# AO33/HiC_Genome_Assembler

Hardware: AMD Instinct MI355X
Metric: Part1+Part2 wall-clock (s) and bins/s on N x N contact map (higher is better)
Workload: dtype f64

## Files before the change

hic_genome_assembler_amd/csrc/api.hip:

```cpp
#include <hip/hip_runtime.h>

#include <algorithm>
#include <cmath>
#include <cstdarg>
#include <climits>
#include <cstdio>
#include <cstdlib>
#include <cstring>
#include <numeric>
#include <string>
#include <type_traits>
#include <unordered_map>
#include <functional>
#include <chrono>
#include <vector>

#include "../../include/hicmi.h"
#include "hicmi_internal.h"
#include "devbuf.h"
#include "hyper.h"

using namespace hicmi;

static thread_local std::string g_err;

static int fail(int code, const char* fmt, ...)
{
    char buf[512];
    va_list ap;
    va_start(ap, fmt);
    vsnprintf(buf, sizeof(buf), fmt, ap);
    va_end(ap);
    g_err = buf;
    return code;
}

namespace hicmi { int set_error(int code, const char* msg) { return fail(code, "%s", msg); } }

#define HIPCHK(expr)                                                                              \
    do {                                                                                          \
        hipError_t _e = (expr);                                                                   \
        if (_e != hipSuccess) return fail(HICMI_EHIP, "%s: %s", #expr, hipGetErrorString(_e));     \
    } while (0)

enum Family { F_ROW_SUMS, F_BUILD_W, F_NNCHAIN, F_SORT, F_RANK_INVERT, F_CUT_COUNT, F_HYPER_FLAGS, F_P2_SELECT,
              F_P2_TOTAL, F_P2_SCORE, F_P2_EXACT, F_P2_INSERT, F_P2_WINDOW_G, F_P2_WINDOW_DELTA, F_PLOT, F_PRESORT, F_RANK_RELABEL,
              F_RANK_TIED, F_P2_WINDOW_FLOPS, F_COUNT };
static const char* kFamilyNames[F_COUNT] = {"row_sums", "build_w", "nnchain", "sort_rows", "rank_invert",
                                            "cut_count", "hyper_flags", "p2_select", "p2_total", "p2_score",
                                            "p2_score_exact", "p2_score_insert", "p2_window_G", "p2_window_delta", "plot",
                                            "presort_rows", "rank_relabel", "rank_rows_tied",
                                            "p2_window_G_flops"};

constexpr int kBaseSlabs = 256;

struct TimedRegion { int fam; hipEvent_t a, b; };

template <typename H, hipError_t (*Destroy)(H)>
struct Handle {
    H h = nullptr;
    Handle() = default;
    Handle(const Handle&) = delete;
    ~Handle() { if (h) (void)Destroy(h); }
    operator H() const { return h; }
};
using StreamHandle = Handle<hipStream_t, hipStreamDestroy>;
using EventHandle = Handle<hipEvent_t, hipEventDestroy>;
struct TimingEvents {
    std::vector<TimedRegion> regions;
    std::vector<hipEvent_t> pool;
    TimingEvents() = default;
    TimingEvents(const TimingEvents&) = delete;
    ~TimingEvents()
    {
        for (auto& r : regions) { (void)hipEventDestroy(r.a); (void)hipEventDestroy(r.b); }
        for (auto e : pool) (void)hipEventDestroy(e);
    }
};

struct hicmi_ctx {
    int device = 0;
    StreamHandle stream;
    StreamHandle stream2; EventHandle ev_fork, ev_join;
    TimingEvents tev;
    int probed_xcc = 0;
    int64_t n = 0, ldc = 0;
    double* dC = nullptr;
    bool own_c = false;
    DevBuf<double> c_own;
    DevBuf<double> d_np, d_seq;
    bool have_sums = false;
    int64_t shard_first = 0, shard_stride = 1;
    DevBuf<double> dW, dW2; int64_t ldw = 0; int64_t w_rows = 0;
    DevBuf<unsigned char> d_size;
    DevBuf<int> d_chain, d_status;
    DevBuf<double> d_zraw;
    std::vector<double> zraw;
    DevBuf<int32_t> d_order;
    DevBuf<uint16_t> dR, dRank; int64_t ldr = 0; int64_t r_rows = 0;
    DevBuf<unsigned char> d_sort_scratch;
    bool have_rank = false;
    DevBuf<uint16_t> dRankS;
    DevBuf<int32_t> d_ident;
    DevBuf<unsigned char> d_ties;
    DevBuf<uint16_t> d_tie_bits; int64_t ld_bits = 0;
    DevBuf<int32_t> d_row_list;
    int64_t scan_first_batch = 0, scan_last_improved = 0;
    int64_t presort_tied_rows = 0;
    int presort_used = 0;
    int64_t presort_n = 0;
    bool presort_dealt = false;
    DevBuf<int32_t> d_x; DevBuf<uint8_t> d_sig;
    DevBuf<unsigned char> d_scan_multi;
    int64_t cached_start = -1;
    DevBuf<double> d_tmp;
    DevBuf<double> dM2; int64_t n2 = 0, ld2 = 0;
    DevBuf<int32_t> d_sel;
    DevBuf<double> d_H;
    DevBuf<int32_t> d_perms;
    DevBuf<double> d_scores;
    DevBuf<double> d_partial;
    DevBuf<double> d_T;
    DevBuf<int32_t> d_scaf_start, d_scaf_len; int64_t n_scaf = 0;
    std::vector<int32_t> h_scaf_start, h_scaf_len;
    DevBuf<int32_t> d_arr_packed;
    std::vector<int32_t> h_arr_packed;
    std::vector<int32_t> h_arr_id, h_arr_pos; std::vector<uint8_t> h_arr_rev;
    DevBuf<int32_t> d_pos2sel; int64_t n_arr = 0;
    DevBuf<int8_t> d_orders; DevBuf<uint8_t> d_orients;
    int tab_k = 0; int64_t n_orders = 0, n_orients = 0;
    std::vector<int8_t> h_orders; std::vector<uint8_t> h_orients;
    std::vector<int32_t> h_pos2sel;
    uint64_t arr_version = 0;
    uint64_t cur_lit_version = ~0ull; double cur_lit_total = 0.0, cur_lit_value = 0.0;
    double cache_total = 0.0; bool cache_valid = false;
    std::unordered_map<std::string, double> exact_cache;
    DevBuf<double> d_G;
    DevBuf<double> d_delta;
    DevBuf<WindowBatchEntry> d_wb;
    int near_min_k = 7;
    DevBuf<unsigned char> d_wnear;
    DevBuf<int32_t> d_arr_packed2;
    DevBuf<int32_t> d_pos2sel2;
    DevBuf<double> d_ins_T;
    DevBuf<double> d_ins_partial;
    DevBuf<unsigned char> d_ins_blob;
    DevBuf<InsStep> d_ins_steps;
    DevBuf<SupRec> d_sup_recs;
    DevBuf<BrkRec> d_brk_recs;
    DevBuf<InvRec> d_inv_recs;
    DevBuf<int32_t> d_gs_lists;
    DevBuf<double> d_gs_sums;
    DevBuf<unsigned char> d_jn_lists;
    DevBuf<double> d_jn_sums;
    DevBuf<double> d_ice;
    DevBuf<uint8_t> d_ice_mask;
    struct HmmSlot { DevBuf<double> d_x; int64_t T = 0, ld = 0, D = 0; };
    HmmSlot hslot[HICMI_HMM_MAX_SLOTS]; int hcur = 0;
    double* d_hx = nullptr; int64_t hmm_T = 0, hmm_ld = 0, hmm_D = 0;
    DevBuf<unsigned char> d_hmulti;
    DevBuf<int32_t> d_horder;
    DevBuf<double> d_hwork;
    DevBuf<int32_t> d_hlab;
    DevBuf<uint8_t> d_hbt;
    DevBuf<double> d_hpart;
    DevBuf<double> d_hsmall;
    DevBuf<double> d_hhist;
    DevBuf<int> d_hst;
    DevBuf<double> d_lvA; int64_t lv_m = 0;
    DevBuf<double> d_lvvec;
    DevBuf<int32_t> d_lvrows;
    DevBuf<unsigned char> d_lvwork;
    DevBuf<double> map_cells; int64_t map_m = 0, map_res = 0, map_pairs = 0;
    DevBuf<int32_t> d_map_first;
    std::vector<int32_t> map_first; std::vector<int64_t> map_size;
    DevBuf<unsigned char> d_map_chunk;
    DevBuf<unsigned char> d_map_lift; LiftTables map_lift; std::vector<int32_t> map_lift_seq;
    DevBuf<unsigned char> d_stat_lift;
    DevBuf<unsigned long long> d_stat_out;
    DevBuf<unsigned long long> span_marks;
    DevBuf<unsigned char> d_span_lift; LiftTables span_lift; SpanGrid span_grid;
    DevBuf<int64_t> d_span_first;
    std::vector<int64_t> span_size, span_seq_first;
    int64_t span_pairs = 0;
    DevBuf<unsigned long long> ends_table; int64_t ends_cells = 0;
    DevBuf<unsigned char> d_ends_lift; LiftTables ends_lift; EndsGrid ends_grid;
    DevBuf<int32_t> d_ends_rank;
    std::vector<int64_t> ends_size;
    DevBuf<unsigned long long> anchor_table; int64_t anchor_cells = 0;
    DevBuf<unsigned char> d_anchor_lift; LiftTables anchor_lift; AnchorGrid anchor_grid;
    DevBuf<int64_t> d_anchor_first;
    DevBuf<int32_t> d_anchor_target;
    std::vector<int64_t> anchor_size;
    DevBuf<int32_t> d_pairs_scaf_a, d_pairs_scaf_b;
    DevBuf<int64_t> d_pairs_pos_a, d_pairs_pos_b;
    DevBuf<unsigned long long> d_pairs_intra;
    DevBuf<long long> d_pairs_work;
    PinBuf<unsigned long long> pin_pairs_len;
    int64_t pairs_len = 0;
    std::vector<int64_t> pairs_size;
    DevBuf<int32_t> d_plot_order;
    DevBuf<unsigned char> d_plot_work;
    DevBuf<double> d_plot_img;
    PinBuf<char> pin_up; size_t pin_up_off = 0;
    PinBuf<char> pin_down;

    int timing = 0;
    double ms[F_COUNT] = {0}; int64_t launches[F_COUNT] = {0}; double bytes[F_COUNT] = {0};
    double nn_scans = 0, nn_scan_cols = 0, nn_cache_hits = 0, nn_merges = 0; int64_t nn_retries = 0;
};

namespace {
hipError_t sync_stream(hicmi_ctx* c);

struct Timed {
    hicmi_ctx* c; int fam; hipEvent_t a = nullptr, b = nullptr; hipStream_t st;
    Timed(hicmi_ctx* ctx, int f, double algo_bytes, hipStream_t on_stream = nullptr) : c(ctx), fam(f), st(on_stream ? on_stream : ctx->stream)
    {
        c->launches[f]++; c->bytes[f] += algo_bytes;
        if (!on()) return;
        a = grab(); b = grab();
        hipEventRecord(a, st);
    }
    bool on() const { return c->timing == 1 || (c->timing == 2 && (fam <= F_RANK_INVERT || fam >= F_PRESORT)); }
    ~Timed()
    {
        if (!on()) return;
        hipEventRecord(b, st);
        c->tev.regions.push_back({fam, a, b});
    }
    hipEvent_t grab()
    {
        if (!c->tev.pool.empty()) { hipEvent_t e = c->tev.pool.back(); c->tev.pool.pop_back(); return e; }
        hipEvent_t e; hipEventCreate(&e); return e;
    }
};

int resolve_timing(hicmi_ctx* c)
{
    if (c->tev.regions.empty()) return HICMI_OK;
    HIPCHK(sync_stream(c));
    if (c->stream2) HIPCHK(hipStreamSynchronize(c->stream2));
    int dropped = 0, dropped_fam = 0;
    hipError_t dropped_err = hipSuccess;
    for (auto& r : c->tev.regions) {
        float ms = 0.f;
        const hipError_t e = hipEventElapsedTime(&ms, r.a, r.b);
        if (e == hipSuccess) c->ms[r.fam] += ms;
        else if (dropped++ == 0) { dropped_fam = r.fam; dropped_err = e; }
        c->tev.pool.push_back(r.a); c->tev.pool.push_back(r.b);
    }
    c->tev.regions.clear();
    if (dropped)
        return fail(HICMI_EHIP, "hipEventElapsedTime failed for %d timed region(s), the first of family %s: %s", dropped,
                    kFamilyNames[dropped_fam], hipGetErrorString(dropped_err));
    return HICMI_OK;
}


hipError_t sync_stream(hicmi_ctx* c)
{
    hipError_t e = hipStreamSynchronize(c->stream);
    c->pin_up_off = 0;
    return e;
}

int upload(hicmi_ctx* c, void* dst, const void* src, size_t bytes)
{
    if (bytes == 0) return HICMI_OK;
    const size_t need = (bytes + 63) & ~(size_t)63;
    if (c->pin_up_off + need > (size_t)c->pin_up.capacity()) {
        HIPCHK(sync_stream(c));
        if (need > (size_t)c->pin_up.capacity()) HIPCHK(c->pin_up.reserve((int64_t)std::max<size_t>(need * 2, (size_t)1 << 20)));
    }
    char* slot = c->pin_up + c->pin_up_off;
    memcpy(slot, src, bytes);
    c->pin_up_off += need;
    HIPCHK(hipMemcpyAsync(dst, slot, bytes, hipMemcpyHostToDevice, c->stream));
    return HICMI_OK;
}

int ensure_pin_down(hicmi_ctx* c, size_t bytes)
{
    if (bytes > (size_t)c->pin_down.capacity()) HIPCHK(c->pin_down.reserve((int64_t)std::max<size_t>(bytes * 2, (size_t)1 << 20)));
    return HICMI_OK;
}

int download(hicmi_ctx* c, void* dst, const void* src, size_t bytes)
{
    if (bytes == 0) { HIPCHK(sync_stream(c)); return HICMI_OK; }
    int rc_pin = ensure_pin_down(c, bytes);
    if (rc_pin) return rc_pin;
    HIPCHK(hipMemcpyAsync(c->pin_down, src, bytes, hipMemcpyDeviceToHost, c->stream));
    HIPCHK(sync_stream(c));
    memcpy(dst, c->pin_down, bytes);
    return HICMI_OK;
}

int no_memory(size_t bytes, hipError_t e)
{
    return fail(HICMI_ENOMEM, "hipMalloc" "(%lld bytes): %s", (long long)bytes, hipGetErrorString(e));
}

template <typename T>
int ensure(DevBuf<T>& buf, int64_t need)
{
    const hipError_t e = buf.reserve(need);
    return e == hipSuccess ? HICMI_OK : no_memory(DevBuf<T>::bytes_for(need), e);
}

template <typename... Args>
int ensure_all(Args&&... args)
{
    size_t failed_bytes = 0;
    const hipError_t e = reserve_all(&failed_bytes, args...);
    return e == hipSuccess ? HICMI_OK : no_memory(failed_bytes, e);
}

int check_candidate_bins(int64_t n_bins)
{
    if (n_bins * (int64_t)sizeof(int32_t) > 160 * 1024) return fail(HICMI_EUNSUPPORTED, "candidate longer than 40960 bins");
    return HICMI_OK;
}

void drop_matrix_state(hicmi_ctx* c)
{
    c->c_own.reset();
    c->dC = nullptr; c->own_c = false; c->n = 0; c->ldc = 0;
    c->d_np.reset(); c->d_seq.reset(); c->have_sums = false;
    c->have_rank = false; c->cached_start = -1; c->n2 = 0;
    if (c->presort_n && c->stream2) (void)hipStreamSynchronize(c->stream2);
    c->presort_n = 0;
}

int alloc_sums(hicmi_ctx* c)
{
    return ensure_all(c->d_np, c->n, c->d_seq, c->n);
}

int compute_sums(hicmi_ctx* c)
{
    if (c->have_sums) return HICMI_OK;
    if (!c->dC) return fail(HICMI_EINVAL, "no contact matrix set");
    {
        Timed t(c, F_ROW_SUMS, 2.0 * 8.0 * (double)c->n * (double)c->n);
        launch_row_sums(c->dC, c->ldc, (int)c->n, c->d_np, c->d_seq, 0, 1, c->stream);
    }
    HIPCHK(hipGetLastError());
    c->have_sums = true;
    return HICMI_OK;
}

int own_matrix(hicmi_ctx* c, DevBuf<double>&& made, int64_t n)
{
    drop_matrix_state(c);
    c->c_own = std::move(made);
    c->dC = c->c_own; c->own_c = true; c->n = n; c->ldc = n;
    int rc = alloc_sums(c);
    return rc ? rc : compute_sums(c);
}

int check_job_context(hicmi_ctx* const* ctxs, int64_t j)
{
    if (!ctxs[j] || !ctxs[0] || ctxs[j]->device != ctxs[0]->device) return fail(HICMI_EINVAL, "contexts must share one device");
    for (int64_t q = 0; q < j; q++) if (ctxs[q] == ctxs[j]) return fail(HICMI_EINVAL, "one context per chromosome");
    return HICMI_OK;
}
}

extern "C" {

int hicmi_abi_version(void) { return HICMI_ABI_VERSION; }
const char* hicmi_last_error(void) { return g_err.c_str(); }

int hicmi_device_count(int* count)
{
    if (!count) return fail(HICMI_EINVAL, "count is NULL");
    int n = 0;
    hipError_t e = hipGetDeviceCount(&n);
    if (e != hipSuccess) { *count = 0; return fail(HICMI_EHIP, "hipGetDeviceCount: %s", hipGetErrorString(e)); }
    *count = n;
    return HICMI_OK;
}

int hicmi_create(int device, hicmi_ctx** out)
{
    if (!out) return fail(HICMI_EINVAL, "out is NULL");
    *out = nullptr;
    int n = 0;
    hipError_t e = hipGetDeviceCount(&n);
    if (e != hipSuccess || n <= 0)
        return fail(HICMI_EHIP, "no HIP device available (%s): libhicmi has no CPU fallback",
                    e != hipSuccess ? hipGetErrorString(e) : "device count 0");
    if (device < 0 || device >= n) return fail(HICMI_EINVAL, "device %d out of range (0..%d)", device, n - 1);
    HIPCHK(hipSetDevice(device));
    hicmi_ctx* c = new hicmi_ctx();
    c->device = device;
    hipError_t se = hipStreamCreateWithFlags(&c->stream.h, hipStreamNonBlocking);
    if (se != hipSuccess) { delete c; return fail(HICMI_EHIP, "hipStreamCreate: %s", hipGetErrorString(se)); }
    c->probed_xcc = nnchain_probe_xcc(c->stream);
    if (const char* dd = getenv("HICMI_P2_DEVICE_DECIDE")) {
        if (!strcmp(dd, "off")) c->near_min_k = INT_MAX;
        else if (atoi(dd) >= 1) c->near_min_k = atoi(dd);
    }
    *out = c;
    return HICMI_OK;
}

int hicmi_destroy(hicmi_ctx* c)
{
    if (!c) return HICMI_OK;
    (void)hipSetDevice(c->device);
    (void)hipStreamSynchronize(c->stream);
    if (c->stream2) (void)hipStreamSynchronize(c->stream2);
    delete c;
    return HICMI_OK;
}

int hicmi_stream(hicmi_ctx* c, void** stream_out)
{
    if (!c || !stream_out) return fail(HICMI_EINVAL, "NULL argument");
    *stream_out = (void*)c->stream;
    return HICMI_OK;
}

int hicmi_synchronize(hicmi_ctx* c)
{
    if (!c) return fail(HICMI_EINVAL, "NULL context");
    HIPCHK(sync_stream(c));
    return HICMI_OK;
}

int hicmi_set_contacts_host(hicmi_ctx* c, const double* contacts, int64_t n)
{
    if (!c || !contacts || n < 1) return fail(HICMI_EINVAL, "bad arguments");
    if (n > 65536) return fail(HICMI_EUNSUPPORTED, "n = %lld > 65536 bins: rank matrix is uint16 in this version", (long long)n);
    HIPCHK(hipSetDevice(c->device));
    drop_matrix_state(c);
    int rc = ensure(c->c_own, n * n);
    if (rc) return rc;
    c->n = n; c->ldc = n; c->dC = c->c_own; c->own_c = true;
    HIPCHK(hipMemcpyAsync(c->dC, contacts, sizeof(double) * (size_t)n * (size_t)n, hipMemcpyHostToDevice, c->stream));
    HIPCHK(sync_stream(c));
    return alloc_sums(c);
}

int hicmi_set_contacts_host_f32(hicmi_ctx* c, const float* contacts, int64_t n)
{
    if (!c || !contacts || n < 1) return fail(HICMI_EINVAL, "bad arguments");
    if (n > 65536) return fail(HICMI_EUNSUPPORTED, "n = %lld > 65536 bins: rank matrix is uint16 in this version", (long long)n);
// ... 2652 lines not shown

void pick_first_strict_max(const std::vector<int64_t>& near, const std::vector<double>& near_fast, const std::vector<double>& lit,
                           double floor, int64_t* pick_out, double* best_out, double* pick_fast_out)
{
    double best = floor; int64_t pick = -1; size_t pick_q = 0;
    for (size_t q = 0; q < near.size(); q++) if (lit[q] > best) { best = lit[q]; pick = near[q]; pick_q = q; }
    *pick_out = pick; *best_out = best;
    if (pick >= 0) *pick_fast_out = near_fast[pick_q];
}

int decide_from_near(hicmi_ctx* c, int64_t first, int64_t k, double total, double floor, double cur_fast, int64_t c0,
                     const std::vector<int64_t>& near, const std::vector<double>& near_fast, int64_t* pick_out,
                     double* best_out, double* pick_fast_out)
{
    const int64_t S = (int64_t)c->h_arr_id.size();
    *pick_out = -1; *best_out = floor; *pick_fast_out = cur_fast;
    if (near.empty()) return HICMI_OK;
    int rc;
    double lit_c0 = 0.0; bool have_c0 = false;
    if (k != S) {
        for (int64_t cand : near) if (cand == c0) have_c0 = true;
        if (have_c0) {
            if (c->cur_lit_version != c->arr_version || c->cur_lit_total != total) {
                std::vector<std::vector<int32_t>> one(1, c->h_pos2sel);
                std::vector<double> v;
                rc = literal_scores(c, one, total, v);
                if (rc) return rc;
                c->cur_lit_version = c->arr_version; c->cur_lit_total = total; c->cur_lit_value = v[0];
            }
            lit_c0 = c->cur_lit_value;
            if (near.size() == 1) {
                if (lit_c0 > floor) { *pick_out = c0; *best_out = lit_c0; *pick_fast_out = near_fast[0]; }
                return HICMI_OK;
            }
        }
    }
    std::vector<int64_t> others;
    for (int64_t cand : near) if (!(have_c0 && cand == c0)) others.push_back(cand);
    std::vector<std::vector<int32_t>> rows;
    near_rows(c, first, k, others, rows);
    std::vector<double> lit_others;
    rc = literal_scores(c, rows, total, lit_others);
    if (rc) return rc;
    std::vector<double> lit(near.size());
    for (size_t q = 0, o = 0; q < near.size(); q++) lit[q] = (have_c0 && near[q] == c0) ? lit_c0 : lit_others[o++];
    pick_first_strict_max(near, near_fast, lit, floor, pick_out, best_out, pick_fast_out);
    return HICMI_OK;
}

int decide_from_delta(hicmi_ctx* c, int64_t first, int64_t k, double total, double floor, double& cur_fast,
                      const double* delta, int64_t* pick_out, double* best_out, double* pick_fast_out)
{
    const int64_t S = (int64_t)c->h_arr_id.size();
    const int64_t n_ord = c->n_orders, n_ori = c->n_orients, n_cand = n_ord * n_ori;
    *pick_out = -1; *best_out = floor; *pick_fast_out = cur_fast;
    const int64_t c0 = window_c0(c, first, k);
    if (c0 < 0) return fail(HICMI_EINVAL, "current orientation not in the orientation table");
    std::vector<double> fast((size_t)n_cand);
    int rc;
    if (k == S) for (int64_t i = 0; i < n_cand; i++) fast[(size_t)i] = delta[(size_t)i] / total;
    else {
        if (std::isnan(cur_fast)) { rc = hicmi_p2_arrangement_score(c, total, &cur_fast); if (rc) return rc; }
        for (int64_t i = 0; i < n_cand; i++) fast[(size_t)i] = cur_fast + (delta[(size_t)i] - delta[(size_t)c0]) / total;
    }
    std::vector<int64_t> near;
    short_list(fast, floor, near);
    std::vector<double> near_fast(near.size());
    for (size_t q = 0; q < near.size(); q++) near_fast[q] = fast[(size_t)near[q]];
    return decide_from_near(c, first, k, total, floor, cur_fast, c0, near, near_fast, pick_out, best_out, pick_fast_out);
}

const int64_t kNearHead = 16;

struct NearPending { int64_t count = 0, cap = 0, head = 0; size_t off_cnt = 0, off_list = 0, host_list = 0; };

int window_near_enqueue(hicmi_ctx* c, int64_t first0, int64_t count, int64_t k, double total, double floor, double& cur_fast,
                        int64_t cap, NearPending& p)
{
    std::vector<WindowBatchEntry> wb;
    BatchCost bc;
    int rc = fill_batch(c, first0, count, k, wb, bc);
    if (rc) return rc;
    if (k > 8 || cap < 1 || cap > (1 << 24)) return fail(HICMI_EINVAL, "short lists take k <= 8 and 1 <= cap <= 2^24");
    const int64_t S = (int64_t)c->h_arr_id.size();
    for (int64_t wdx = 0; wdx < count; wdx++) {
        const int64_t c0 = window_c0(c, first0 + wdx, k);
        if (c0 < 0) return fail(HICMI_EINVAL, "current orientation not in the orientation table");
        wb[(size_t)wdx].c0 = (int32_t)c0;
    }
    if (k != S && std::isnan(cur_fast)) { rc = hicmi_p2_arrangement_score(c, total, &cur_fast); if (rc) return rc; }
    HIPCHK(hipSetDevice(c->device));
    const int n_blocks = window_near_blocks((int)c->n_orders);
    const size_t off_cnt = (size_t)count * (size_t)n_blocks * sizeof(double);
    const size_t off_list = off_cnt + (((size_t)count * sizeof(int32_t) + 15) & ~(size_t)15);
    const size_t bytes = off_list + (size_t)count * (size_t)cap * sizeof(NearEntry);
    rc = ensure(c->d_G, count * window_table_doubles((int)k));
    if (!rc) rc = ensure(c->d_wnear, (int64_t)bytes);
    if (!rc) rc = ensure(c->d_wb, count);
    if (rc) return rc;
    rc = upload(c, c->d_wb, wb.data(), sizeof(WindowBatchEntry) * (size_t)count);
    if (rc) return rc;
    int32_t* d_count = reinterpret_cast<int32_t*>(c->d_wnear + off_cnt);
    NearEntry* d_list = reinterpret_cast<NearEntry*>(c->d_wnear + off_list);
    {
        c->launches[F_P2_WINDOW_FLOPS]++; c->bytes[F_P2_WINDOW_FLOPS] += bc.g_flops;
        Timed t(c, F_P2_WINDOW_G, bc.g_bytes);
        launch_p2_window_near(c->dM2, c->ld2, c->d_pos2sel, (int)c->n_arr, (int)k, c->d_wb, wb.data(), (int)count, bc.max_m,
                              c->d_orders, c->d_orients, (int)c->n_orders, (int)c->n_orients, c->d_H, c->d_G, k == S ? 1 : 0,
                              total, cur_fast, floor, kNearTop, reinterpret_cast<double*>(c->d_wnear.get()), d_count,
                              d_list, (int)cap, c->stream);
    }
    HIPCHK(hipGetLastError());
    p.count = count; p.cap = cap; p.head = std::min<int64_t>(kNearHead, cap); p.off_cnt = off_cnt; p.off_list = off_list;
    p.host_list = off_list - off_cnt;
    const size_t row = (size_t)p.head * sizeof(NearEntry);
    rc = ensure_pin_down(c, p.host_list + row * (size_t)count);
    if (rc) return rc;
    if (count == 1)
        HIPCHK(hipMemcpyAsync(c->pin_down, d_count, p.host_list + row, hipMemcpyDeviceToHost, c->stream));
    else {
        HIPCHK(hipMemcpyAsync(c->pin_down, d_count, sizeof(int32_t) * (size_t)count, hipMemcpyDeviceToHost, c->stream));
        HIPCHK(hipMemcpy2DAsync(c->pin_down + p.host_list, row, d_list, (size_t)cap * sizeof(NearEntry), row, (size_t)count,
                                hipMemcpyDeviceToHost, c->stream));
    }
    return HICMI_OK;
}

int window_near_collect(hicmi_ctx* c, const NearPending& p, std::vector<int64_t>& n_near,
                        std::vector<std::vector<int64_t>>& near, std::vector<std::vector<double>>& near_fast)
{
    const int64_t count = p.count, cap = p.cap;
    HIPCHK(sync_stream(c));
    std::vector<int32_t> cnt((size_t)count);
    memcpy(cnt.data(), c->pin_down, sizeof(int32_t) * (size_t)count);
    n_near.assign((size_t)count, 0); near.assign((size_t)count, {}); near_fast.assign((size_t)count, {});
    int64_t widest = 0;
    for (int64_t w = 0; w < count; w++) {
        n_near[(size_t)w] = cnt[(size_t)w];
        if (cnt[(size_t)w] <= cap) widest = std::max<int64_t>(widest, cnt[(size_t)w]);
    }
    if (widest == 0) return HICMI_OK;
    size_t row = (size_t)p.head * sizeof(NearEntry);
    const char* lists = c->pin_down + p.host_list;
    if (widest > p.head) {
        row = (size_t)widest * sizeof(NearEntry);
        int rc = ensure_pin_down(c, row * (size_t)count);
        if (rc) return rc;
        HIPCHK(hipMemcpy2DAsync(c->pin_down, row, c->d_wnear + p.off_list, (size_t)cap * sizeof(NearEntry), row, (size_t)count,
                                hipMemcpyDeviceToHost, c->stream));
        HIPCHK(sync_stream(c));
        lists = c->pin_down;
    }
    std::vector<NearEntry> ent;
    for (int64_t w = 0; w < count; w++) {
        const int64_t m = cnt[(size_t)w];
        if (m < 1 || m > cap) continue;
        const NearEntry* src = reinterpret_cast<const NearEntry*>(lists + row * (size_t)w);
        ent.assign(src, src + m);
        std::sort(ent.begin(), ent.end(), [](const NearEntry& a, const NearEntry& b) { return a.cand < b.cand; });
        near[(size_t)w].resize((size_t)m); near_fast[(size_t)w].resize((size_t)m);
        for (int64_t q = 0; q < m; q++) { near[(size_t)w][(size_t)q] = ent[(size_t)q].cand; near_fast[(size_t)w][(size_t)q] = ent[(size_t)q].fast; }
    }
    return HICMI_OK;
}

int window_near_batch(hicmi_ctx* c, int64_t first0, int64_t count, int64_t k, double total, double floor, double& cur_fast,
                      int64_t cap, std::vector<int64_t>& n_near, std::vector<std::vector<int64_t>>& near,
                      std::vector<std::vector<double>>& near_fast)
{
    NearPending p;
    int rc = window_near_enqueue(c, first0, count, k, total, floor, cur_fast, cap, p);
    if (rc) return rc;
    return window_near_collect(c, p, n_near, near, near_fast);
}

const int64_t kNearCap = 4096;

int check_window_call(hicmi_ctx* c, int64_t first, int64_t k)
{
    const int64_t S = (int64_t)c->h_arr_id.size();
    if (c->n_arr < 1 || S < 1) return fail(HICMI_EINVAL, "hicmi_p2_set_arrangement has not run");
    if (k != c->tab_k || c->h_orders.empty()) return fail(HICMI_EINVAL, "hicmi_p2_window_tables has not been called for k = %lld", (long long)k);
    if (first < 0 || first + k > S) return fail(HICMI_EINVAL, "window out of range");
    for (int64_t j = 0; j < k; j++) if (c->h_orders[(size_t)j] != j) return fail(HICMI_EINVAL, "orders[0] must be the identity");
    return HICMI_OK;
}
}

int hicmi_p2_decide_window(hicmi_ctx* c, int64_t first, int64_t k, double total, double floor, double cur_fast,
                           int64_t* pick_out, double* best_out, double* pick_fast_out)
{
    if (!c || !pick_out || !best_out || !pick_fast_out) return fail(HICMI_EINVAL, "NULL argument");
    int rc = check_window_call(c, first, k);
    if (rc) return rc;
    use_total(c, total);
    if (k >= c->near_min_k) {
        std::vector<int64_t> n_near; std::vector<std::vector<int64_t>> near; std::vector<std::vector<double>> near_fast;
        rc = window_near_batch(c, first, 1, k, total, floor, cur_fast, kNearCap, n_near, near, near_fast);
        if (rc) return rc;
        if (n_near[0] <= kNearCap)
            return decide_from_near(c, first, k, total, floor, cur_fast, window_c0(c, first, k), near[0], near_fast[0],
                                    pick_out, best_out, pick_fast_out);
    }
    std::vector<double> delta((size_t)(c->n_orders * c->n_orients));
    rc = window_batch(c, first, 1, k, delta.data());
    if (rc) return rc;
    return decide_from_delta(c, first, k, total, floor, cur_fast, delta.data(), pick_out, best_out, pick_fast_out);
}

int hicmi_p2_window_shortlist(hicmi_ctx* c, int64_t first, int64_t count, int64_t k, double total, double floor,
                              double cur_fast, int64_t cap, int64_t* n_near_out, int64_t* idx_out, double* fast_out)
{
    if (!c || !n_near_out || !idx_out || !fast_out || count < 1) return fail(HICMI_EINVAL, "bad arguments");
    int rc = check_window_call(c, first, k);
    if (rc) return rc;
    std::vector<int64_t> n_near; std::vector<std::vector<int64_t>> near; std::vector<std::vector<double>> near_fast;
    rc = window_near_batch(c, first, count, k, total, floor, cur_fast, cap, n_near, near, near_fast);
    if (rc) return rc;
    for (int64_t w = 0; w < count; w++) {
        n_near_out[w] = n_near[(size_t)w];
        for (size_t q = 0; q < near[(size_t)w].size(); q++) {
            idx_out[w * cap + (int64_t)q] = near[(size_t)w][q];
            fast_out[w * cap + (int64_t)q] = near_fast[(size_t)w][q];
        }
    }
    return HICMI_OK;
}

int hicmi_p2_decide_insertion(hicmi_ctx* c, const int32_t* ids, const uint8_t* rev, int64_t S, int32_t new_id,
                              int32_t new_rev_now, int64_t* gap_out, int32_t* rev_out, double* best_out)
{
    if (!c || !ids || !rev || !gap_out || !rev_out || !best_out || S < 1) return fail(HICMI_EINVAL, "bad arguments");
    if (c->n_scaf < 1) return fail(HICMI_EINVAL, "hicmi_p2_layout has not run");
    if (new_id < 0 || new_id >= c->n_scaf) return fail(HICMI_EINVAL, "new scaffold out of range");
    *gap_out = -1; *rev_out = 0; *best_out = 0.0;
    std::vector<int32_t> ids2(ids, ids + S); ids2.push_back(new_id);
    std::vector<uint8_t> rev2(rev, rev + S); rev2.push_back(new_rev_now ? 1 : 0);
    int rc = hicmi_p2_set_arrangement(c, ids2.data(), rev2.data(), S + 1);
    if (rc) return rc;
    double total = 0.0;
    rc = hicmi_p2_arrangement_total(c, &total);
    if (rc) return rc;
    use_total(c, total);
    rc = hicmi_p2_set_arrangement(c, ids, rev, S);
    if (rc) return rc;
    const int64_t gaps = S + 1;
    std::vector<double> by_gap_rev((size_t)(2 * gaps));
    rc = hicmi_p2_score_insertions(c, new_id, total, by_gap_rev.data());
    if (rc) return rc;
    std::vector<double> fast((size_t)(2 * gaps));
    std::vector<int32_t> tag_rev((size_t)(2 * gaps));
    int32_t o = new_rev_now ? 1 : 0;
    for (int64_t i = 0; i < gaps; i++) {
        tag_rev[(size_t)(2 * i)] = o; tag_rev[(size_t)(2 * i + 1)] = o ^ 1;
        fast[(size_t)(2 * i)] = by_gap_rev[(size_t)(2 * i + o)];
        fast[(size_t)(2 * i + 1)] = by_gap_rev[(size_t)(2 * i + (o ^ 1))];
        o ^= 1;
    }
    std::vector<int64_t> near;
    short_list(fast, 0.0, near);
    if (near.empty()) return HICMI_OK;
    const int32_t st = c->h_scaf_start[(size_t)new_id], ln = c->h_scaf_len[(size_t)new_id];
    std::vector<std::vector<int32_t>> rows(near.size());
    for (size_t q = 0; q < near.size(); q++) {
        const int64_t g = near[q] / 2;
        const int32_t r = tag_rev[(size_t)near[q]];
        const int P = c->h_arr_pos[(size_t)g];
        std::vector<int32_t>& row = rows[q];
        row.reserve((size_t)(c->n_arr + ln));
        row.insert(row.end(), c->h_pos2sel.begin(), c->h_pos2sel.begin() + P);
        if (r) for (int32_t e = 0; e < ln; e++) row.push_back(st + ln - 1 - e);
        else   for (int32_t e = 0; e < ln; e++) row.push_back(st + e);
        row.insert(row.end(), c->h_pos2sel.begin() + P, c->h_pos2sel.end());
    }
    std::vector<double> lit;
    rc = literal_scores(c, rows, total, lit);
    if (rc) return rc;
    double best = 0.0; int64_t pick = -1;
    for (size_t q = 0; q < near.size(); q++) if (lit[q] > best) { best = lit[q]; pick = near[q]; }
    if (pick >= 0) { *gap_out = pick / 2; *rev_out = tag_rev[(size_t)pick]; *best_out = best; }
    return HICMI_OK;
}


namespace {
void apply_insertion(int32_t* ids, uint8_t* rev, int64_t& S, int64_t gap, int32_t new_id, int32_t r)
{
    for (int64_t j = S; j > gap; j--) { ids[j] = ids[j - 1]; rev[j] = rev[j - 1]; }
    ids[gap] = new_id; rev[gap] = (uint8_t)(r ? 1 : 0);
    S++;
}

struct InsJob {
    hicmi_ctx* c; int32_t* ids; uint8_t* rev; int64_t S; const int32_t* new_ids; int64_t n_new;
    int64_t t = 0; double best = 0.0; bool device_ok = true;
};

int queue_insertions(hicmi_ctx* lead, const std::vector<InsJob*>& jobs)
{
    const int nj = (int)jobs.size();
    if (nj == 0) return HICMI_OK;
    const int NB = kBaseSlabs;
    static const int max_c = getenv("HICMI_P2_INS_MAXC") ? atoi(getenv("HICMI_P2_INS_MAXC")) : INS_MAXC;
    int64_t steps_max = 0;
    std::vector<size_t> blob_off((size_t)nj);
    size_t blob_bytes = 0;
    for (int j = 0; j < nj; j++) {
        InsJob& job = *jobs[(size_t)j];
        hicmi_ctx* c = job.c;
        int rc = hicmi_p2_set_arrangement(c, job.ids, job.rev, job.S);
        if (rc) return rc;
        if (c != lead) HIPCHK(sync_stream(c));
        const int64_t n_steps = job.n_new - job.t;
        int64_t n_max = c->n_arr;
        for (int64_t t = 0; t < n_steps; t++) n_max += c->h_scaf_len[(size_t)job.new_ids[job.t + t]];
        rc = check_candidate_bins(n_max);
        if (rc) return rc;
        const int64_t S_max = job.S + n_steps;
        rc = ensure(c->d_arr_packed2, 3 * std::max<int64_t>(S_max, c->n_scaf) + 2);
        if (!rc) rc = ensure(c->d_pos2sel2, c->n2);
        if (!rc) rc = ensure(c->d_ins_T, (1 + 2 * (int64_t)INS_MAXC) * n_max);
        if (!rc) rc = ensure(c->d_ins_partial, NB + n_max + 2 * (S_max + 1));
        if (rc) return rc;
        steps_max = std::max(steps_max, n_steps);
        blob_off[(size_t)j] = blob_bytes;
        blob_bytes += (sizeof(InsState) + sizeof(InsLog) * (size_t)n_steps + 15) & ~(size_t)15;
    }
    HIPCHK(hipSetDevice(lead->device));
    int rc = ensure(lead->d_ins_blob, (int64_t)blob_bytes);
    if (!rc) rc = ensure(lead->d_ins_steps, steps_max * nj);
    if (rc) return rc;
    std::vector<InsStep> table((size_t)(steps_max * nj));
    std::vector<int> max_n_used((size_t)steps_max, 0), max_S((size_t)steps_max, 0), max_n_arr((size_t)steps_max, 0);
    double algo = 0.0;
    for (int j = 0; j < nj; j++) {
        InsJob& job = *jobs[(size_t)j];
        hicmi_ctx* c = job.c;
        const int64_t n_steps = job.n_new - job.t;
        int64_t n_max = c->n_arr;
        for (int64_t t = 0; t < n_steps; t++) n_max += c->h_scaf_len[(size_t)job.new_ids[job.t + t]];
        InsState* st = reinterpret_cast<InsState*>(lead->d_ins_blob + blob_off[(size_t)j]);
        InsLog* log = reinterpret_cast<InsLog*>(lead->d_ins_blob + blob_off[(size_t)j] + sizeof(InsState));
        int32_t* packed[2] = {c->d_arr_packed, c->d_arr_packed2};
        int32_t* pos2sel[2] = {c->d_pos2sel, c->d_pos2sel2};
        int64_t n_arr = c->n_arr;
        for (int64_t t = 0; t < steps_max; t++) {
            InsStep& d = table[(size_t)(t * nj + j)];
            memset(&d, 0, sizeof(d));
            d.st = st;
            if (t >= n_steps) continue;
            const int cur = (int)(t & 1), nxt = cur ^ 1;
            const int32_t nid = job.new_ids[job.t + t];
            const int L = c->h_scaf_len[(size_t)nid];
            d.M2 = c->dM2; d.H = c->d_H; d.ld2 = c->ld2;
            d.pos_cur = pos2sel[cur]; d.pos_nxt = pos2sel[nxt]; d.packed_cur = packed[cur]; d.packed_nxt = packed[nxt];
            d.T_total = c->d_ins_T; d.T_cand = c->d_ins_T + n_max; d.work = c->d_ins_T + (1 + (int64_t)INS_MAXC) * n_max;
            d.partial = c->d_ins_partial; d.log = log + t;
            d.n_arr = (int32_t)n_arr; d.S = (int32_t)(job.S + t); d.L = L; d.new_start = c->h_scaf_start[(size_t)nid];
            d.new_id = nid; d.active = 1; d.step = (int32_t)t; d.last = t == n_steps - 1;
            max_n_used[(size_t)t] = std::max(max_n_used[(size_t)t], (int)(n_arr + L));
            max_S[(size_t)t] = std::max(max_S[(size_t)t], d.S);
            max_n_arr[(size_t)t] = std::max(max_n_arr[(size_t)t], (int)n_arr);
            const double nn = (double)n_arr, Ld = (double)L, sd = (double)d.S;
            algo += 8.0 * (0.5 * nn * (nn - 1.0) + nn * nn + 2.0 * (sd + 1.0) * Ld * nn) + 4.0 * (nn + Ld) * (nn + Ld);
            n_arr += L;
        }
    }
    rc = upload(lead, lead->d_ins_steps, table.data(), sizeof(InsStep) * table.size());
    if (rc) return rc;
    {
        Timed timed(lead, F_P2_INSERT, algo);
        launch_insb_reset(lead->d_ins_steps, nj, lead->stream);
        for (int64_t t = 0; t < steps_max; t++) {
            const InsStep* st_t = lead->d_ins_steps + t * nj;
            const int nu = max_n_used[(size_t)t];
            launch_insb_fast(st_t, nj, max_S[(size_t)t], max_n_arr[(size_t)t], NB, lead->stream);
            launch_insb_shortlist(st_t, nj, max_S[(size_t)t], max_n_arr[(size_t)t], NB, kNearTop, max_c, lead->stream);
            launch_insb_diag_cand(st_t, nj, nu, lead->stream);
            launch_insb_cost(st_t, nj, nu, lead->stream);
            launch_insb_apply(st_t, nj, nu, lead->stream);
        }
    }
    HIPCHK(hipGetLastError());
    std::vector<unsigned char> blob(blob_bytes);
    rc = download(lead, blob.data(), lead->d_ins_blob, blob_bytes);
    if (rc) return rc;
    if (getenv("HICMI_PART2_PROFILE")) {
        int64_t hist[5] = {0, 0, 0, 0, 0}, all_direct = 0;
        for (int64_t t = 0; t < steps_max; t++) {
            int mx = -1, ran = 0;
            for (int j = 0; j < nj; j++) {
                if (t >= jobs[(size_t)j]->n_new - jobs[(size_t)j]->t) continue;
                const InsState* hs = reinterpret_cast<const InsState*>(blob.data() + blob_off[(size_t)j]);
                if (hs->fail >= 0 && t >= hs->fail) continue;
                const InsLog* hl = reinterpret_cast<const InsLog*>(blob.data() + blob_off[(size_t)j] + sizeof(InsState));
                const int ns = hl[t].n_short;
                hist[ns < 0 ? 0 : (ns > 3 ? 4 : ns + 1)]++;
                mx = std::max(mx, ns);
                ran++;
            }
            if (ran && mx < 0) all_direct++;
        }
        fprintf(stderr, "[hicmi] insertion short lists: direct %lld, literal with 0:%lld 1:%lld 2:%lld 3+:%lld candidates; "
                        "lock steps without any literal pass: %lld of %lld\n",
                (long long)hist[0], (long long)hist[1], (long long)hist[2], (long long)hist[3], (long long)hist[4],
                (long long)all_direct, (long long)steps_max);
    }
    for (int j = 0; j < nj; j++) {
        InsJob& job = *jobs[(size_t)j];
        const int64_t n_steps = job.n_new - job.t;
        const InsState* hst = reinterpret_cast<const InsState*>(blob.data() + blob_off[(size_t)j]);
        const InsLog* hlog = reinterpret_cast<const InsLog*>(blob.data() + blob_off[(size_t)j] + sizeof(InsState));
        const int64_t done = hst->fail >= 0 ? std::min<int64_t>(hst->fail, n_steps) : n_steps;
        for (int64_t t = 0; t < done; t++) {
            if (hlog[t].gap < 0 || hlog[t].gap > job.S) return fail(HICMI_ESTATE, "insertion log out of range");
            apply_insertion(job.ids, job.rev, job.S, hlog[t].gap, job.new_ids[job.t + t], hlog[t].rev);
            job.best = hlog[t].best;
        }
        job.t += done;
        hicmi_ctx* c = job.c;
        c->n_arr = 0; c->h_arr_id.clear(); c->h_arr_rev.clear(); c->h_arr_pos.clear(); c->h_pos2sel.clear();
    }
    return HICMI_OK;
}

int check_insert_job(const InsJob& job, int64_t S0)
{
    hicmi_ctx* c = job.c;
    if (!c || !job.ids || !job.rev || !job.new_ids || S0 < 1 || job.n_new < 1) return fail(HICMI_EINVAL, "bad arguments");
    if (c->n_scaf < 1) return fail(HICMI_EINVAL, "hicmi_p2_layout has not run");
    std::vector<uint8_t> used((size_t)c->n_scaf, 0);
    for (int64_t j = 0; j < S0 + job.n_new; j++) {
        const int32_t v = j < S0 ? job.ids[j] : job.new_ids[j - S0];
        if (v < 0 || v >= c->n_scaf || used[(size_t)v]) return fail(HICMI_EINVAL, "scaffolds must be distinct members of the layout");
        used[(size_t)v] = 1;
    }
    return HICMI_OK;
}

int host_insertion_step(InsJob& job)
{
    int64_t gap = -1; int32_t r = 0;
    int rc = hicmi_p2_decide_insertion(job.c, job.ids, job.rev, job.S, job.new_ids[job.t], 0, &gap, &r, &job.best);
    if (rc) return rc;
    if (gap < 0) { gap = 0; r = 0; job.best = 0.0; }
    apply_insertion(job.ids, job.rev, job.S, gap, job.new_ids[job.t], r);
    job.t++;
    return HICMI_OK;
}

int run_insert_jobs(std::vector<InsJob>& all)
{
    static const bool host_only = getenv("HICMI_P2_HOST_INSERT") != nullptr;
    for (InsJob& job : all) {
        int rc = check_insert_job(job, job.S);
        if (rc) return rc;
        if (job.S + job.n_new + 1 > 8192) job.device_ok = false;
    }
    while (true) {
        std::vector<InsJob*> todo;
        for (InsJob& job : all) if (job.t < job.n_new && job.device_ok && !host_only) todo.push_back(&job);
        if (!todo.empty()) {
            int rc = queue_insertions(todo[0]->c, todo);
            if (rc) return rc;
        }
        bool pending = false;
        for (InsJob& job : all) {
            if (job.t >= job.n_new) continue;
            do {
                int rc = host_insertion_step(job);
                if (rc) return rc;
            } while (job.t < job.n_new && (host_only || !job.device_ok));
            if (job.t < job.n_new) pending = true;
        }
        if (!pending) break;
    }
    return HICMI_OK;
}
}

int hicmi_p2_insert_all(hicmi_ctx* c, int32_t* ids, uint8_t* rev, int64_t S0, const int32_t* new_ids, int64_t n_new,
                        double* best_out)
{
    if (!c || !best_out) return fail(HICMI_EINVAL, "bad arguments");
    std::vector<InsJob> jobs(1);
    jobs[0].c = c; jobs[0].ids = ids; jobs[0].rev = rev; jobs[0].S = S0; jobs[0].new_ids = new_ids; jobs[0].n_new = n_new;
    int rc = run_insert_jobs(jobs);
    if (rc) return rc;
    *best_out = jobs[0].best;
    return HICMI_OK;
}

int hicmi_p2_insert_all_multi(int64_t n_jobs, hicmi_ctx* const* ctxs, int32_t* const* ids, uint8_t* const* rev,
                              const int64_t* S0, const int32_t* const* new_ids, const int64_t* n_new, double* best_out)
{
    if (n_jobs < 1 || !ctxs || !ids || !rev || !S0 || !new_ids || !n_new || !best_out) return fail(HICMI_EINVAL, "bad arguments");
    std::vector<InsJob> jobs((size_t)n_jobs);
    for (int64_t j = 0; j < n_jobs; j++) {
        InsJob& job = jobs[(size_t)j];
        job.c = ctxs[j]; job.ids = ids[j]; job.rev = rev[j]; job.S = S0[j]; job.new_ids = new_ids[j]; job.n_new = n_new[j];
        if (int rc = check_job_context(ctxs, j)) return rc;
    }
    int rc = run_insert_jobs(jobs);
    if (rc) return rc;
    for (int64_t j = 0; j < n_jobs; j++) best_out[j] = jobs[(size_t)j].best;
    return HICMI_OK;
}

extern "C++" {
namespace {
template <typename Rec>
struct TableOps {
    int64_t max_S;
    DevBuf<Rec> hicmi_ctx::*recs;
    std::function<void(int64_t j, int64_t& n_table, int64_t& scratch, int64_t& n_rec)> size;
    std::function<int(int64_t j, double* d_scores, int32_t* d_best, std::vector<Rec>& recs, double& algo)> append;
    std::function<void(const Rec* d_recs, int n_rec)> launch;
};

template <typename Rec>
int run_table_jobs(int64_t n_jobs, hicmi_ctx* const* ctxs, const int32_t* const* ids, const uint8_t* const* rev,
                   const int64_t* S, const double* totals, double* const* scores_out, int32_t* const* best_out,
                   const TableOps<Rec>& ops)
{
    hicmi_ctx* lead = ctxs[0];
    std::vector<size_t> out_off((size_t)n_jobs, 0);
    std::vector<int64_t> n_table((size_t)n_jobs, 0);
    std::vector<uint8_t> run((size_t)n_jobs, 0);
    size_t blob_bytes = 0;
    int64_t n_rec = 0;
    for (int64_t j = 0; j < n_jobs; j++) {
        int rc = check_job_context(ctxs, j);
        if (rc) return rc;
        hicmi_ctx* c = ctxs[j];
        if (!ids[j] || !rev[j] || !scores_out[j] || !best_out[j] || S[j] < 1) return fail(HICMI_EINVAL, "bad arguments");
        if (ops.max_S && S[j] > ops.max_S) return fail(HICMI_EUNSUPPORTED, "more than %d scaffolds in one chromosome", (int)ops.max_S);
        rc = hicmi_p2_set_arrangement(c, ids[j], rev[j], S[j]);
        if (rc) return rc;
        if (c != lead) HIPCHK(sync_stream(c));
        rc = check_candidate_bins(c->n_arr);
        if (rc) return rc;
        int64_t scratch = 0, n_rec_j = 0;
        ops.size(j, n_table[(size_t)j], scratch, n_rec_j);
        for (int64_t i = 0; i < n_table[(size_t)j]; i++) scores_out[j][i] = 0.0;
        for (int64_t i = 0; i < S[j]; i++) { best_out[j][2 * i] = -1; best_out[j][2 * i + 1] = 0; }
        if (c->n_arr < 2 || !(totals[j] > 0.0) || n_rec_j == 0) continue;
        run[(size_t)j] = 1;
        rc = ensure(c->d_ins_partial, scratch);
        if (rc) return rc;
        out_off[(size_t)j] = blob_bytes;
        blob_bytes += ((size_t)n_table[(size_t)j] * sizeof(double) + (size_t)(2 * S[j]) * sizeof(int32_t) + 15) & ~(size_t)15;
        n_rec += n_rec_j;
    }
    if (n_rec == 0) return HICMI_OK;
    HIPCHK(hipSetDevice(lead->device));
    int rc = ensure(lead->d_ins_blob, (int64_t)blob_bytes);
    if (!rc) rc = ensure(lead->*ops.recs, n_rec);
    if (rc) return rc;
    std::vector<Rec> recs;
    recs.reserve((size_t)n_rec);
    double algo = 0.0;
    for (int64_t j = 0; j < n_jobs; j++) {
        if (!run[(size_t)j]) continue;
        double* d_scores = reinterpret_cast<double*>(lead->d_ins_blob + out_off[(size_t)j]);
        rc = ops.append(j, d_scores, reinterpret_cast<int32_t*>(d_scores + n_table[(size_t)j]), recs, algo);
        if (rc) return rc;
    }
    rc = upload(lead, lead->*ops.recs, recs.data(), sizeof(Rec) * recs.size());
    if (rc) return rc;
    {
        Timed timed(lead, F_P2_INSERT, algo);
        ops.launch(lead->*ops.recs, (int)n_rec);
    }
    HIPCHK(hipGetLastError());
    std::vector<unsigned char> blob(blob_bytes);
    rc = download(lead, blob.data(), lead->d_ins_blob, blob_bytes);
    if (rc) return rc;
    for (int64_t j = 0; j < n_jobs; j++) {
        if (!run[(size_t)j]) continue;
        const size_t nd = (size_t)n_table[(size_t)j];
        memcpy(scores_out[j], blob.data() + out_off[(size_t)j], nd * sizeof(double));
        memcpy(best_out[j], blob.data() + out_off[(size_t)j] + nd * sizeof(double), (size_t)(2 * S[j]) * sizeof(int32_t));
    }
    return HICMI_OK;
}
}
}

int hicmi_p2_support_multi(int64_t n_jobs, hicmi_ctx* const* ctxs, const int32_t* const* ids, const uint8_t* const* rev,
                           const int64_t* S, const double* totals, double* const* scores_out, int32_t* const* best_out)
{
    if (n_jobs < 1 || !ctxs || !ids || !rev || !S || !totals || !scores_out || !best_out) return fail(HICMI_EINVAL, "bad arguments");
    const int NB = SUP_BASE_SLABS;
    int max_S = 1, max_n = 1;
    TableOps<SupRec> ops;
    ops.max_S = SUP_MAX_S; ops.recs = &hicmi_ctx::d_sup_recs;
    ops.size = [&](int64_t j, int64_t& n_table, int64_t& scratch, int64_t& n_rec) {
        n_table = 2 * S[j] * S[j]; scratch = S[j] * (NB + ctxs[j]->n_arr + 2 * S[j]); n_rec = S[j];
    };
    ops.append = [&](int64_t j, double* d_scores, int32_t* d_best, std::vector<SupRec>& recs, double& algo) {
        hicmi_ctx* c = ctxs[j];
        const int64_t Sj = S[j], n = c->n_arr;
        max_S = std::max(max_S, (int)Sj);
        max_n = std::max(max_n, (int)n);
        for (int64_t k = 0; k < Sj; k++) {
            SupRec d;
            memset(&d, 0, sizeof(d));
            const int32_t sid = ids[j][k];
            d.M2 = c->dM2; d.H = c->d_H; d.ld2 = c->ld2;
            d.pos = c->d_pos2sel; d.arr_pos = c->d_arr_packed + Sj;
            d.partial = c->d_ins_partial + k * (NB + n + 2 * Sj);
            d.scores = d_scores + 2 * Sj * k; d.best = d_best + 2 * k;
            d.total = totals[j];
            d.n = (int32_t)n; d.S = (int32_t)Sj; d.j = (int32_t)k;
            d.start = c->h_scaf_start[(size_t)sid]; d.L = c->h_scaf_len[(size_t)sid]; d.cur_rev = rev[j][k] ? 1 : 0;
            recs.push_back(d);
            const double nn = (double)(n - d.L);
            algo += 8.0 * (0.5 * nn * nn + nn * nn + 2.0 * (double)Sj * (double)d.L * nn);
        }
        return (int)HICMI_OK;
    };
    ops.launch = [&](const SupRec* d_recs, int n_rec) { launch_sup(d_recs, n_rec, max_S, max_n, kNearTop, ctxs[0]->stream); };
    return run_table_jobs(n_jobs, ctxs, ids, rev, S, totals, scores_out, best_out, ops);
}

int hicmi_p2_support(hicmi_ctx* c, const int32_t* ids, const uint8_t* rev, int64_t S, double total, double* scores_out,
                     int32_t* best_out)
{
    return hicmi_p2_support_multi(1, &c, &ids, &rev, &S, &total, &scores_out, &best_out);
}

int hicmi_p2_breaks_multi(int64_t n_jobs, hicmi_ctx* const* ctxs, const int32_t* const* ids, const uint8_t* const* rev,
                          const int64_t* S, const double* totals, int64_t min_piece, double* const* scores_out,
                          int32_t* const* best_out)
{
    if (n_jobs < 1 || !ctxs || !ids || !rev || !S || !totals || !scores_out || !best_out || min_piece < 1)
        return fail(HICMI_EINVAL, "bad arguments");
    const int NB = BRK_BASE_SLABS;
    int64_t n_wg = 0;
    TableOps<BrkRec> ops;
    ops.max_S = 0; ops.recs = &hicmi_ctx::d_brk_recs;
    ops.size = [&](int64_t j, int64_t& n_table, int64_t& scratch, int64_t& n_rec) {
        scratch = NB;
        for (int64_t k = 0; k < S[j]; k++) {
            const int64_t L = ctxs[j]->h_scaf_len[(size_t)ids[j][k]];
            if (L < 2) continue;
            n_table += 8 * (L - 1); scratch += L * L + 3 * (L - 1); n_rec++;
        }
    };
    ops.append = [&](int64_t j, double* d_scores, int32_t* d_best, std::vector<BrkRec>& recs, double& algo) {
        hicmi_ctx* c = ctxs[j];
        const int64_t Sj = S[j], n = c->n_arr;
        int rc = upload(ctxs[0], d_best, best_out[j], sizeof(int32_t) * (size_t)(2 * Sj));
        if (rc) return rc;
        double* scratch = c->d_ins_partial + NB;
        int64_t row = 0;
        bool first = true;
        for (int64_t k = 0; k < Sj; k++) {
            const int64_t L = c->h_scaf_len[(size_t)ids[j][k]];
            if (L < 2) continue;
            BrkRec d;
            memset(&d, 0, sizeof(d));
            d.M2 = c->dM2; d.H = c->d_H; d.ld2 = c->ld2;
            d.pos = c->d_pos2sel;
            d.X = scratch; d.pq = scratch + L * L; scratch += L * L + 3 * (L - 1);
            d.base = c->d_ins_partial;
            d.scores = d_scores + 8 * row; d.best = d_best + 2 * k; row += L - 1;
            d.total = totals[j];
            d.wg0 = n_wg;
            d.n = (int32_t)n; d.B = c->h_arr_pos[(size_t)k]; d.L = (int32_t)L;
            d.min_piece = (int32_t)std::min<int64_t>(min_piece, 1 << 30);
            d.n_base = first ? NB : 0;
            first = false;
            n_wg += d.n_base + L * ((L + 3) / 4) + (L - 1);
            recs.push_back(d);
            algo += 8.0 * ((double)L * (double)L * (double)(n - L) + (double)L * (double)L * (double)L / 6.0);
        }
        algo += 4.0 * (double)n * (double)n;
        if (n_wg > 0x7fffffff) return fail(HICMI_EUNSUPPORTED, "more than 2^31 - 1 workgroups in one call");
        return (int)HICMI_OK;
    };
    ops.launch = [&](const BrkRec* d_recs, int n_rec) { launch_brk(d_recs, n_rec, n_wg, kNearTop, ctxs[0]->stream); };
    return run_table_jobs(n_jobs, ctxs, ids, rev, S, totals, scores_out, best_out, ops);
// ... 1024 lines not shown
```

hic_genome_assembler_amd/csrc/hicmi_internal.h:

```cpp
#pragma once
#include <hip/hip_runtime.h>
#include <stdint.h>

#include <atomic>
#include <functional>

#include "liftmap.h"
#include "span.h"
#include "ends.h"
#include "anchor.h"
#include "pairs.h"
#include "split.h"

namespace hicmi {

inline void ensure_dynamic_lds(const void* func, std::atomic<int>& have, size_t bytes)
{
    if ((int)bytes > have.load(std::memory_order_relaxed)) {
        (void)hipFuncSetAttribute(func, hipFuncAttributeMaxDynamicSharedMemorySize, (int)bytes);
        have.store((int)bytes, std::memory_order_relaxed);
    }
}

static constexpr int SERIAL_BATCH = 16;

__device__ __forceinline__ double serial_sum_lds(const double* t, int from, int to, double acc)
{
    constexpr int B = SERIAL_BATCH;
    int i = from;
    if (i + B <= to) {
        double a[B];
#pragma unroll
        for (int q = 0; q < B; q++) a[q] = t[i + q];
        while (i + 2 * B <= to) {
            double b[B];
#pragma unroll
            for (int q = 0; q < B; q++) b[q] = t[i + B + q];
#pragma unroll
            for (int q = 0; q < B; q++) acc += a[q];
#pragma unroll
            for (int q = 0; q < B; q++) a[q] = b[q];
            i += B;
        }
#pragma unroll
        for (int q = 0; q < B; q++) acc += a[q];
        i += B;
    }
    for (; i < to; i++) acc += t[i];
    return acc;
}

__device__ __forceinline__ double serial_prefix_lds(double* t, int from, int to, double acc)
{
    constexpr int B = SERIAL_BATCH;
    int i = from;
    if (i + B <= to) {
        double a[B];
#pragma unroll
        for (int q = 0; q < B; q++) a[q] = t[i + q];
        while (i + 2 * B <= to) {
            double b[B];
#pragma unroll
            for (int q = 0; q < B; q++) b[q] = t[i + B + q];
#pragma unroll
            for (int q = 0; q < B; q++) { acc += a[q]; t[i + q] = acc; }
#pragma unroll
            for (int q = 0; q < B; q++) a[q] = b[q];
            i += B;
        }
#pragma unroll
        for (int q = 0; q < B; q++) { acc += a[q]; t[i + q] = acc; }
        i += B;
    }
    for (; i < to; i++) { acc += t[i]; t[i] = acc; }
    return acc;
}

static constexpr int MAX_LEAVES = 65;

__device__ __forceinline__ int enumerate_leaves(int off, int len, int* leaf_off, int* leaf_len, int* leaf_dep,
                                                int* st_off, int* st_len, int* st_dep)
{
    int sp = 1, n = 0;
    st_off[0] = off; st_len[0] = len; st_dep[0] = 0;
    while (sp > 0) {
        sp--;
        const int o = st_off[sp], l = st_len[sp], d = st_dep[sp];
        if (l <= 128) { leaf_off[n] = o; leaf_len[n] = l; leaf_dep[n] = d; n++; continue; }
        int n2 = l / 2;
        n2 -= n2 % 8;
        st_off[sp] = o + n2; st_len[sp] = l - n2; st_dep[sp] = d + 1; sp++;
        st_off[sp] = o; st_len[sp] = n2; st_dep[sp] = d + 1; sp++;
    }
    return n;
}

__device__ __forceinline__ double combine_leaves(int n_leaves, const double* leaf_sum, const int* leaf_dep, double* val,
                                                 int* dep)
{
    int sp = 0;
    for (int l = 0; l < n_leaves; l++) {
        double v = leaf_sum[l];
        int d = leaf_dep[l];
        while (sp > 0 && dep[sp - 1] == d) { v = val[sp - 1] + v; d--; sp--; }
        val[sp] = v; dep[sp] = d; sp++;
    }
    return val[0];
}

void launch_row_sums(const double* C, int64_t ldc, int n, double* np_sum, double* seq_sum, int row_first, int row_stride,
                     hipStream_t s);
void launch_pairwise_rows(const double* C, int64_t ldc, int len, int rows, double* out, hipStream_t s);
void launch_compact(const double* src, int64_t ld_src, const int32_t* keep, int n_keep, double* dst, int64_t ld_dst,
                    hipStream_t s);
void launch_widen_f32(const float* src, double* dst, int64_t cells, hipStream_t s);
void launch_build_w(const double* C, int64_t ldc, const double* np_sum, int n, double* W, int64_t ldw, hipStream_t s);
size_t nnchain_workspace_bytes(int n);
struct NNChainOptions {
    bool profile = false;
    int dcap = 256;
    bool dcap_forced = false;
    bool compact = true;
    bool wgs_set = false; int wgs = 0;
    bool plain = false;
    bool gsize = false;
    bool w1 = true;
    int w1_s = 0;
    int w1_cols = 0;
    int w1_maxs = 0;
    int xcc = -1;
    int test_late = 0, test_diverge = 0, test_rollcall = 0;
};
NNChainOptions nnchain_options(int probed_xcc);
int nnchain_probe_xcc(hipStream_t s);
int launch_nnchain(double* W, double* W2, int64_t ldw, int n, int* chain, double* zraw, void* workspace, const NNChainOptions& o,
                   int fallback, hipStream_t s, const std::function<void()>& after_first_rowmin = nullptr);
void launch_selftest_division(unsigned long long seed, int blocks, int iters, unsigned long long* d_mismatches, hipStream_t s);
const int* nnchain_state_ptr(void* workspace);
const unsigned long long* nnchain_prof_ptr(void* workspace);
void launch_cut_count(const uint16_t* rank, int64_t ldr, int row0, int nrows, int lo, int mode, int cparam,
                      int32_t* x_out, int row_step, hipStream_t s);
void launch_hyper_flags(const int32_t* x, int nrows, int mode, int L_fixed, int64_t M, double psig, uint8_t* sig,
                        int own_first, int own_step, hipStream_t s);

struct ScanState {
    int done;
    int mode;
    int start, cut, n_rows, recount;
    long long M;
    double psig;
    int min_size, stop_ind, loop_count, n_cuts, n_log, scans;
    int MD, n_alt, alt_off, f_i, f_keep_from, f_noise, f_round, f_max_rounds, f_warned;
    int pad;
    unsigned long long bytes;
};
static constexpr int SCAN_MAX_SETS = 64;
void launch_first_pass_multi_pairs(const uint16_t* rank, int64_t ldr, int n, int n_sets, ScanState* st, int32_t* x, uint8_t* sig,
                                   double psig0, int share, int32_t* cuts, int32_t* mlog, int log_cap, int pairs, hipStream_t s);
void launch_filter_multi_pairs(const uint16_t* rank, int64_t ldr, int n, int max_rows, int n_sets, ScanState* st, int32_t* x,
                               uint8_t* sig, double psig0, int share, int32_t* alt, uint8_t* filt, uint8_t* prev,
                               int32_t* seg, int32_t* seg_x, int pairs, hipStream_t s);

#if defined(__HIPCC__)
template <int M>
__device__ __forceinline__ uint32_t xor_lane(uint32_t v, int lane)
{
    if constexpr (M == 1) return (uint32_t)__builtin_amdgcn_mov_dpp((int)v, 0xB1, 0xf, 0xf, true);
    else if constexpr (M == 2) return (uint32_t)__builtin_amdgcn_mov_dpp((int)v, 0x4E, 0xf, 0xf, true);
    else if constexpr (M == 4) {
        const int t = __builtin_amdgcn_mov_dpp((int)v, 0x141, 0xf, 0xf, true);
        return (uint32_t)__builtin_amdgcn_mov_dpp(t, 0x1B, 0xf, 0xf, true);
    } else if constexpr (M == 8) {
        const int t = __builtin_amdgcn_mov_dpp((int)v, 0x140, 0xf, 0xf, true);
        return (uint32_t)__builtin_amdgcn_mov_dpp(t, 0x141, 0xf, 0xf, true);
    } else if constexpr (M == 16) {
        const auto r = __builtin_amdgcn_permlane16_swap(v, v, false, false);
        return (lane & 16) ? r[0] : r[1];
    } else {
        static_assert(M == 32, "xor_lane: M must be 1, 2, 4, 8, 16 or 32");
        const auto r = __builtin_amdgcn_permlane32_swap(v, v, false, false);
        return (lane & 32) ? r[0] : r[1];
    }
}
#endif

int  sort_padded_size(int n);
int  sort_workgroups(int n);
size_t sort_scratch_bytes(int n);
struct SortExtras {
    const int32_t* row_list = nullptr; int n_list = 0;
    uint8_t* tie_flag = nullptr; unsigned* tie_count = nullptr; unsigned tie_limit = 0;
    uint16_t* tie_bits = nullptr; int64_t ld_bits = 0;
    int max_workgroups = 0;
    int avoid_xcc = -1; unsigned* row_counter = nullptr;
};
static constexpr int GETREG_XCC_ID = 20 | (0 << 6) | (3 << 11);
int nnchain_local_xcc(const NNChainOptions& o, int n);
void launch_sort_rows(const double* C, int64_t ldc, const int32_t* order, const int32_t* inv, const double* np_sum,
                      const double* seq_sum, int n, void* scratch, uint16_t* R, int64_t ldr, int row_first, int row_stride,
                      hipStream_t s, const SortExtras& x = SortExtras());
void launch_rank_rows_tied(const uint16_t* R_storage, const uint16_t* tie_bits, int64_t ld_bits, const int32_t* order,
                           const int32_t* inv, int n, const int32_t* row_list, int n_list, uint16_t* rank, int64_t ldr,
                           hipStream_t s, int32_t* done = nullptr);
void launch_rank_relabel(const uint16_t* rank_storage, uint16_t* rank, int64_t ldr, int n, const int32_t* order, int row_first,
                         int row_stride, hipStream_t s);
size_t sort_radix_scratch_bytes(int n);
void launch_rank_rows_radix(const double* C, int64_t ldc, const int32_t* order, const int32_t* inv, const double* np_sum,
                            const double* seq_sum, int n, void* scratch, uint16_t* rank, int64_t ldr, int row_first,
                            int row_stride, hipStream_t s);
void launch_rank_invert(const uint16_t* R, uint16_t* rank, int64_t ldr, int n, int row_first, int row_stride, hipStream_t s,
                        const int32_t* row_list = nullptr, int n_list = 0);
void launch_similarity_row(const double* C, int64_t ldc, const int32_t* order, const double* np_sum,
                           const double* seq_sum, int n, int row, double* out, hipStream_t s);

void launch_p2_select(const double* C, int64_t ldc, const int32_t* sel, int n, double* M2, int64_t ld2, hipStream_t s);
void launch_p2_total(const double* M2, int64_t ld2, int n, double* T, double* total, hipStream_t s);
void launch_p2_score_exact(const double* M2, int64_t ld2, const int32_t* perms, int n_cand, int n_used, double total,
                           double* T, double* work, double* scores, hipStream_t s);
void launch_p2_score(const double* M2, int64_t ld2, const int32_t* perms, int n_cand, int n_used, const double* H,
                     double inv_total_unused, double total, double* scores, hipStream_t s);

void launch_p2_total_perm(const double* M2, int64_t ld2, const int32_t* d_perm, int n, double* T, double* total,
                          hipStream_t s);

struct WindowDesc {
    int32_t start[8];
    int32_t len[8];
    int32_t off[8];
    uint8_t rev[8];
};
void launch_arr_materialize(const int32_t* packed, int S, const int32_t* scaf_start, const int32_t* scaf_len, int n_arr,
                            int32_t* pos2sel, hipStream_t s);
void launch_p2_base_partial(const double* M2, int64_t ld2, const int32_t* pos2sel, int n_arr, const double* H, int n_tot,
                            int n_blocks, double* out, hipStream_t s);
void launch_p2_insert_delta(const double* M2, int64_t ld2, const int32_t* pos2sel, int n_arr, const int32_t* arr_pos,
                            int S, int new_start, int L, const double* H, int n_base_blocks, double* out, hipStream_t s);
struct WindowBatchEntry {
    WindowDesc w;
    int32_t p0, m;
    int64_t g_off;
    int32_t c0, pad;
};
void launch_p2_window_batch_G(const double* M2, int64_t ld2, const int32_t* pos2sel, int n, const WindowBatchEntry* wb, int n_win,
                              int max_m, const double* H, double* G_all, hipStream_t s);
void launch_p2_window_batch_delta(const double* M2, int64_t ld2, const int32_t* pos2sel, int n, int k,
                                  const WindowBatchEntry* wb, int n_win, int max_m, const int8_t* orders, const uint8_t* orients,
                                  int n_ord, int n_ori, const double* H, const double* G_all, double* delta_all, hipStream_t s);


int64_t window_table_doubles(int k);
void launch_p2_window_tables(const double* M2, int64_t ld2, const int32_t* pos2sel, int n, int k,
                             const WindowBatchEntry* wb, const WindowBatchEntry* h_wb, int n_win, int max_m, const double* H,
                             double* tables, hipStream_t s);
void launch_p2_window_candidates(int k, int n_win, const int8_t* orders, const uint8_t* orients, int n_ord, int n_ori,
                                 const double* tables, double* delta_all, hipStream_t s);
struct NearEntry { int32_t cand, pad; double fast; };
int window_near_blocks(int n_ord);
void launch_p2_window_near(const double* M2, int64_t ld2, const int32_t* pos2sel, int n, int k,
                           const WindowBatchEntry* wb, const WindowBatchEntry* h_wb, int n_win, int max_m, const int8_t* orders,
                           const uint8_t* orients, int n_ord, int n_ori, const double* H, double* tables, int whole, double total,
                           double cur_fast, double floor, double near_top, double* part, int32_t* count, NearEntry* near, int cap,
                           hipStream_t s);

__device__ __forceinline__ double wave_sum_s(double v)
{
#pragma unroll
    for (int off = 32; off >= 1; off >>= 1) v += __shfl_xor(v, off, 64);
    return v;
}

__device__ __forceinline__ double block_sum_256(double v, double* s_w)
{
    v = wave_sum_s(v);
    if ((threadIdx.x & 63) == 0) s_w[threadIdx.x >> 6] = v;
    __syncthreads();
    return (s_w[0] + s_w[1]) + (s_w[2] + s_w[3]);
}

__device__ __forceinline__ void base_partial_body(const double* __restrict__ M2, int64_t ld2, const int32_t* p, int n_arr,
                                                  const double* __restrict__ H, int n_tot, int blk, int n_blk,
                                                  double* __restrict__ out)
{
    __shared__ double s_w[4];
    const int lane = threadIdx.x & 63, wave = threadIdx.x >> 6;
    const double hn = H[n_tot - 1];
    double acc = 0.0;
    for (int a = blk * 4 + wave; a < n_arr - 1; a += n_blk * 4) {
        const double* __restrict__ row = M2 + (int64_t)p[a] * ld2;
#pragma unroll 4
        for (int b = a + 1 + lane; b < n_arr; b += 64) acc += row[p[b]] * (hn - H[b - a - 1]);
    }
    double sum = block_sum_256(acc, s_w);
    if (threadIdx.x == 0) out[0] = sum;
}

template <typename Counts>
__device__ __forceinline__ void pick_first_max_256(int tid, int n_cand, const double* scores, int32_t* best,
                                                   double near_top, Counts counts)
{
    __shared__ double s_val[256];
    __shared__ int s_idx[256], s_cnt;
    double mx = -__builtin_inf();
    int at = 0x7fffffff;
    for (int i = tid; i < n_cand; i += 256) {
        const double v = scores[i];
        if (counts(i) && isfinite(v) && v > mx) { mx = v; at = i; }
    }
    s_val[tid] = mx; s_idx[tid] = at;
    if (tid == 0) s_cnt = 0;
    __syncthreads();
    for (int w = 128; w >= 1; w >>= 1) {
        if (tid < w) {
            const double o = s_val[tid + w];
            const int oi = s_idx[tid + w];
            if (o > s_val[tid] || (o == s_val[tid] && oi < s_idx[tid])) { s_val[tid] = o; s_idx[tid] = oi; }
        }
        __syncthreads();
    }
    const double top = s_val[0];
    const int first = s_idx[0];
    if (first == 0x7fffffff) {
        if (tid == 0) { best[0] = -1; best[1] = 0; }
        return;
    }
    const double thr = top - fabs(top) * near_top;
    int near = 0;
    for (int i = tid; i < n_cand; i += 256) {
        const double v = scores[i];
        near += counts(i) && isfinite(v) && v >= thr;
    }
    if (near) atomicAdd(&s_cnt, near);
    __syncthreads();
    if (tid == 0) { best[0] = first; best[1] = s_cnt; }
}

static constexpr int INS_MAXC = 8;
struct InsState {
    int32_t fail;
    int32_t n_short;
    int32_t direct, pad;
    int32_t gap[INS_MAXC], rev[INS_MAXC], idx[INS_MAXC];
    double total;
    double lit[INS_MAXC];
};
struct InsLog { int32_t gap, rev; double best; int32_t n_short, pad; };
struct InsStep {
    const double* M2; const double* H; int64_t ld2;
    const int32_t* pos_cur; int32_t* pos_nxt;
    const int32_t* packed_cur; int32_t* packed_nxt;
    double *T_total, *T_cand, *work, *partial;
    InsState* st; InsLog* log;
    int32_t n_arr, S, L, new_start, new_id, active, step, last;
};
void launch_insb_reset(const InsStep* steps, int n_chrom, hipStream_t s);
void launch_insb_fast(const InsStep* steps, int n_chrom, int max_S, int max_n_arr, int n_base_blocks, hipStream_t s);
void launch_insb_shortlist(const InsStep* steps, int n_chrom, int max_S, int max_n_arr, int n_base_blocks, double near_top,
                           int max_c, hipStream_t s);
void launch_insb_diag_cand(const InsStep* steps, int n_chrom, int max_n_used, hipStream_t s);
void launch_insb_cost(const InsStep* steps, int n_chrom, int max_n_used, hipStream_t s);
void launch_insb_apply(const InsStep* steps, int n_chrom, int max_n_used, hipStream_t s);

static constexpr int SUP_BASE_SLABS = 64;
static constexpr int SUP_MAX_S = 4096;
struct SupRec {
    const double* M2; const double* H; int64_t ld2;
    const int32_t* pos;
    const int32_t* arr_pos;
    double* partial;
    double* scores;
    int32_t* best;
    double total;
    int32_t n, S, j, start, L, cur_rev;
};
void launch_sup(const SupRec* recs, int n_rec, int max_S, int max_n, double near_top, hipStream_t s);

static constexpr int BRK_BASE_SLABS = 64;
struct BrkRec {
    const double* M2; const double* H; int64_t ld2;
    const int32_t* pos;
    double* X;
    double* pq;
    double* base;
    double* scores;
    int32_t* best;
    double total;
    int64_t wg0;
    int32_t n, B, L, min_piece;
    int32_t n_base, pad;
};
void launch_brk(const BrkRec* recs, int n_rec, int64_t n_wg, double near_top, hipStream_t s);

static constexpr int INV_BASE_SLABS = 64;
static constexpr int INV_MAX_S = 4096;
static constexpr double INV_MAX_WORK = 1e13;
struct InvRec {
    const double* M2; const double* H; int64_t ld2;
    const int32_t* pos;
    const int32_t* arr_pos;
    double* base;
    double* scores;
    int32_t* best;
    double total;
    int64_t wg0;
    int32_t n, S, i, n_j;
    int32_t max_span, n_base;
};
void launch_inv(const InvRec* recs, int n_rec, int64_t n_wg, double near_top, hipStream_t s);

static constexpr int GS_CHUNK = 64;
struct GsChunk { int32_t row0, cnt, group, pad; };
void launch_group_sums(const double* C, int64_t ld, int n, int G, int S, const int32_t* rows, const GsChunk* chunks,
                       int n_chunks, const int32_t* group_chunk0, const int32_t* scaf, const int32_t* sbins,
                       const int32_t* soff, double* partial, double* binsum, double* scafsum, bool plain, hipStream_t s);

static constexpr int JN_SLAB_ROWS = 64;
struct JnRec {
    int64_t wg0;
    int32_t startA, stepA, lenA;
    int32_t startB, stepB, lenB;
    int32_t n_slabs, pad;
};
void launch_junction_sums(const double* C, int64_t ld, const int32_t* bins, const JnRec* recs, int n_rec, int64_t n_wg,
                          const double* w, double* partial, double* sums, bool plain, hipStream_t s);

void launch_ice_fill(double* v, int n, double value, hipStream_t s);
void launch_ice_rowdot(const double* C, int64_t ld, int n, const double* u, double* y, hipStream_t s);
void launch_ice_vec_b(int n, const double* y, double* u, double* bias, double* prev, double* sums, double* st,
                      double* rec, int it, int first, hipStream_t s);
void launch_ice_vec_a(int n, const double* sums, double* bias, double* u, double* d, hipStream_t s);
void launch_ice_apply(double* X, int64_t ld, int n, const double* u, hipStream_t s);
void launch_ice_scale(double* X, int64_t ld, int n, const double* d, const double* st, int by_c, hipStream_t s);
void launch_ice_mask(double* X, int64_t ld, int n, const uint8_t* mask, hipStream_t s);

static constexpr int REBIN_MAX_WIDTH = 64;
static constexpr int REBIN_CHUNK = 1024;
void launch_rebin(const double* C, int64_t ld, int n, const int32_t* group_start, const int32_t* chunk_first, int m,
                  double* R, bool plain, hipStream_t s);

static constexpr int BUILDMAP_SLICE = 2048;
static constexpr int BUILDMAP_SLOTS = 4096;
static constexpr int PAIRSTATS_SLICE = 1024;
static constexpr int PAIRSTATS_SLOT_BITS = 12;
static constexpr int PAIRSTATS_SLOTS = 1 << PAIRSTATS_SLOT_BITS;
void launch_buildmap_add(const int32_t* scaf_a, const int64_t* pos_a, const int32_t* scaf_b, const int64_t* pos_b, int64_t n,
                         const int32_t* first_bin, int n_grid, int64_t r, int m, void* counts, bool plain, const LiftTables& lift,
                         hipStream_t s);
void launch_pair_stats(const int32_t* scaf_a, const int64_t* pos_a, const int32_t* scaf_b, const int64_t* pos_b, int64_t n,
                       const LiftTables& lift, void* out, hipStream_t s);
void launch_buildmap_finish(void* cells, int m, hipStream_t s);

static constexpr int SPAN_SLICE = 2048;
static constexpr int SPAN_SLOT_BITS = 11;
static constexpr int SPAN_SLOTS = 1 << SPAN_SLOT_BITS;
static constexpr int SPAN_PROBES = 8;
static constexpr int SPAN_SCAN_ITEMS = 8;
static constexpr int SPAN_SCAN_TILE = 2048;
static constexpr int SPAN_SCAN_WIDTH = 1024;
void launch_span_mark(const int32_t* scaf_a, const int64_t* pos_a, const int32_t* scaf_b, const int64_t* pos_b, int64_t n,
                      const LiftTables& lift, const SpanGrid& grid, void* marks, void* counters, bool plain, hipStream_t s);
int64_t span_scan_tiles(int64_t n);
void launch_span_scan(const void* in, void* out, int64_t n, void* tile_sums, hipStream_t s);
void launch_span_pick(const void* depth, const void* depth_sums, int64_t n_cells, int64_t flank, const int64_t* recs, int64_t n_rec,
                      int64_t* picks, hipStream_t s);

static constexpr int ENDS_SLICE = 2048;
static constexpr int ENDS_SLOT_BITS = 10;
static constexpr int ENDS_SLOTS = 1 << ENDS_SLOT_BITS;
static constexpr int ENDS_PROBES = 8;
void launch_ends_count(const int32_t* scaf_a, const int64_t* pos_a, const int32_t* scaf_b, const int64_t* pos_b, int64_t n,
                       const LiftTables& lift, const EndsGrid& grid, int64_t n_table, void* table, void* counters, bool plain,
                       hipStream_t s);

static constexpr int ANCHOR_SLICE = 2048;
static constexpr int ANCHOR_SLOT_BITS = 10;
static constexpr int ANCHOR_SLOTS = 1 << ANCHOR_SLOT_BITS;
static constexpr int ANCHOR_PROBES = 8;
void launch_anchor_count(const int32_t* scaf_a, const int64_t* pos_a, const int32_t* scaf_b, const int64_t* pos_b, int64_t n,
                         const LiftTables& lift, const AnchorGrid& grid, int64_t n_table, void* table, void* counters, bool plain,
                         hipStream_t s);

static constexpr int PAIRS_SLICE = 2048;
static constexpr int PAIRS_SLOT_BITS = 8;
static constexpr int PAIRS_SLOTS = 1 << PAIRS_SLOT_BITS;
static constexpr int PAIRS_PROBES = 8;
struct PairStore { int32_t* scaf_a = nullptr; int64_t* pos_a = nullptr; int32_t* scaf_b = nullptr; int64_t* pos_b = nullptr; int64_t cap = 0; };
int64_t pairs_keep_blocks(int64_t n);
void launch_pairs_keep(const int32_t* scaf_a, const int64_t* pos_a, const int32_t* scaf_b, const int64_t* pos_b, int64_t n,
                       int64_t n_scaf, const PairStore& store, void* length, void* intra, void* work, bool plain, hipStream_t s);

static constexpr int SPLIT_SLICE = 2048;
static constexpr int SPLIT_SLOT_BITS = 11;
static constexpr int SPLIT_SLOTS = 1 << SPLIT_SLOT_BITS;
static constexpr int SPLIT_PROBES = 8;
static constexpr int SPLIT_MAX_BLOCKS = 1024;
void launch_split_pairs(int32_t* scaf_a, int64_t* pos_a, int32_t* scaf_b, int64_t* pos_b, int64_t n, const SplitTables& tables,
                        void* counters, bool plain, hipStream_t s);

void launch_plot_select(const double* C, int64_t ldc, const double* np_sum, const double* seq_sum, int kind,
                        const int32_t* order, int n_sel, int n_targets, struct SelectState* d_state, unsigned int* d_hist,
                        hipStream_t s);
size_t plot_select_state_bytes();
size_t plot_select_hist_bytes();
int plot_select_max_targets();
void plot_select_fill(void* host_state, const unsigned long long* ranks, int n_targets);
double plot_select_value(const void* host_state, int t);
void launch_plot_downsample(const double* C, int64_t ldc, const double* np_sum, const double* seq_sum, int kind,
                            const int32_t* order, int n_sel, int px, double* out, hipStream_t s);

enum { HMM_P_MEAN = 0, HMM_P_VAR = 2, HMM_P_MOV = 4, HMM_P_IV = 6, HMM_P_LOGV = 8, HMM_P_MU2V = 10, HMM_P_SCALARS = 12 };
enum { HMM_S_CONST = 0, HMM_S_A = 2, HMM_S_LOGA = 6, HMM_S_PI = 10, HMM_S_LOGPI = 12, HMM_S_XI = 14, HMM_S_POST = 18,
       HMM_S_COUNT = 32 };
int  hmm_col_chunks(int T, int D);
__host__ __device__ inline void hmm_col_shape(int T, int R, int& rows_per, int& Rr)
{
    rows_per = (T + R - 1) / R;
    Rr = (T + rows_per - 1) / rows_per;
}
struct HmmKmProb {
    const double* X; int64_t ld; int T, D;
    int nc, rows_per, Rr, max_iter;
    int64_t rows[2];
    double tol;
    double *cen, *sums, *part, *out;
    int32_t* lab;
};
enum { HMM_KM_LLOYD = 0, HMM_KM_FINAL = 1, HMM_KM_SUM = 2, HMM_KM_DONE = 3 };
struct HmmKmState { int phase, cur, it, strict, changed, n1; double inertia; };
void launch_hmm_obs(const double* C, int64_t ldc, const int32_t* order, const double* np_sum, const double* seq_sum,
                    int c, int T, int D, double* X, hipStream_t s);
void launch_hmm_colsum(int mode, const double* X, int64_t ld, int T, int D, const double* shift, const int32_t* labels,
                       const double* g, double* part, double* out, hipStream_t s);
void launch_hmm_dist2(const double* X, int64_t ld, int T, int D, const double* cen, int nc, double* dist, hipStream_t s);
void launch_hmm_assign(const double* X, int64_t ld, int T, int D, const double* cen, const int32_t* old_labels,
                       int32_t* labels, double* mind, int* st, hipStream_t s);
void launch_hmm_center_update(const double* sums, int T, int D, const int* st, double* cen, double* shift_out, hipStream_t s);
void launch_hmm_sum(const double* v, int n, double* out, hipStream_t s);
void launch_hmm_params(const double* sums, int D, int from_sums, double* P, hipStream_t s);
void launch_hmm_emission(const double* X, int64_t ld, int T, int D, const double* P, double* L, hipStream_t s);
void launch_hmm_fb(const double* L, int T, double* P, int D, double* alpha, double* beta, double* gam, double* hist, int it,
                   hipStream_t s);
void launch_hmm_viterbi(const double* L, int T, const double* P, int D, uint8_t* bt, int32_t* states, hipStream_t s);
void launch_hmm_multi_seed(const HmmKmProb* pr, HmmKmState* st, int n_prob, int max_rows, int kmeans, hipStream_t s);
void launch_hmm_dist2_multi(const HmmKmProb* pr, int n_prob, int max_T, hipStream_t s);
void launch_hmm_kmeans_multi_step(const HmmKmProb* pr, HmmKmState* st, int* done, int n_prob, int max_T, int max_items,
                                  int max_2d, hipStream_t s);

static constexpr int LOUVAIN_MAX_M = 16384;
static constexpr int LOUVAIN_MAX_ROUNDS = 1024;
__host__ __device__ inline size_t louvain_round_bytes(int m) { return (size_t)m * (4 * sizeof(double) + 8 * sizeof(int)); }
int  louvain_level0_lds_max();
void launch_louvain_graph(const double* C, int64_t ldc, const int32_t* rows, const double* np_sum, const double* seq_sum, int m,
                          double* A, hipStream_t s);
void launch_louvain_status(const double* A, int m, double* diag, double* rowsum, double* chunk, double* dsum, double* gdeg,
                           double* total, hipStream_t s);
void launch_louvain_level0(const double* A, int m, const double* gdeg, const double* loops, const double* total, int rounds,
                           const uint64_t* st_in, int32_t* n2c_out, uint64_t* st_out, int32_t* info, double* deg_out,
                           double* int_out, unsigned char* scratch, hipStream_t s);
void launch_louvain_induced(const double* A, int m, const int32_t* members, const int32_t* moff, int k, double* rowagg,
                            double* B, hipStream_t s);
void launch_louvain_score(const double* A, int m, const int32_t* parts, int rounds, const double* gdeg, const double* total,
                          double* same, double* acc, double* q, hipStream_t s);

}
```

hic_genome_assembler_amd/csrc/k_part2.hip:

```cpp
#include <cstdlib>

#include "hicmi_internal.h"

namespace hicmi {

__global__ __launch_bounds__(256) void k_p2_select(const double* __restrict__ C, int64_t ldc,
                                                   const int32_t* __restrict__ sel, int n, double* __restrict__ M2,
                                                   int64_t ld2)
{
    int r = blockIdx.y;
    int c = blockIdx.x * 256 + threadIdx.x;
    if (c >= n) return;
    M2[(int64_t)r * ld2 + c] = C[(int64_t)sel[r] * ldc + sel[c]];
}

void launch_p2_select(const double* C, int64_t ldc, const int32_t* sel, int n, double* M2, int64_t ld2, hipStream_t s)
{
    hipLaunchKernelGGL(k_p2_select, dim3((n + 255) / 256, n), dim3(256), 0, s, C, ldc, sel, n, M2, ld2);
}

__device__ __forceinline__ double wave_sum(double v)
{
#pragma unroll
    for (int off = 32; off >= 1; off >>= 1) v += __shfl_xor(v, off, 64);
    return v;
}


struct IndexMap {
    const int32_t* p;
    int P, L, new_start, rev;
    __device__ __forceinline__ int at(int t) const
    {
        if (t < P) return p ? p[t] : t;
        if (t - P < L) return new_start + (rev ? L - 1 - (t - P) : t - P);
        return p ? p[t - L] : t - L;
    }
};
static constexpr int kNoSplice = 0x7fffffff;

__device__ __forceinline__ int diag_of_block(int b) { return ((((b >> 6) << 3) + (b & 7)) << 3) + ((b >> 3) & 7) + 1; }
static int diag_grid(int n_used) { return ((n_used - 1) + 63) & ~63; }

__device__ __forceinline__ double diag_sum_body(const double* __restrict__ M2, int64_t ld2, const IndexMap& m, int n_used,
                                                int off)
{
    __shared__ int leaf_off[MAX_LEAVES], leaf_len[MAX_LEAVES], leaf_dep[MAX_LEAVES];
    __shared__ double leaf_sum[MAX_LEAVES];
    __shared__ int s_nleaves, st_a[16], st_b[16], st_c[16];
    __shared__ double st_v[16];
    const int lane = threadIdx.x, slot = lane >> 3, k = lane & 7;
    const int len = n_used - off;
    auto elem = [&](int t) -> double { return M2[(int64_t)m.at(t) * ld2 + m.at(t + off)]; };
    double acc = 0.0;
    for (int c0 = 0; c0 < len; c0 += 8192) {
        const int clen = len - c0 < 8192 ? len - c0 : 8192;
        __syncthreads();
        if (lane == 0) s_nleaves = enumerate_leaves(c0, clen, leaf_off, leaf_len, leaf_dep, st_a, st_b, st_c);
        __syncthreads();
        const int nl = s_nleaves;
        for (int l0 = 0; l0 < nl; l0 += 8) {
            const int l = l0 + slot;
            double r = 0.0;
            int o = 0, n = 0, lim = 0;
            if (l < nl) { o = leaf_off[l]; n = leaf_len[l]; lim = n - (n % 8); }
            {
                int64_t idx[16];
                double vals[16];
#pragma unroll
                for (int q = 0; q < 16; q++) {
                    const bool ok = l < nl && n >= 8 && q * 8 < lim;
                    const int t = o + q * 8 + k;
                    const int a = ok ? m.at(t) : 0, b = ok ? m.at(t + off) : 0;
                    idx[q] = (int64_t)a * ld2 + b;
                }
#pragma unroll
                for (int q = 0; q < 16; q++) vals[q] = (l < nl && n >= 8 && q * 8 < lim) ? M2[idx[q]] : 0.0;
                r = vals[0];
#pragma unroll
                for (int q = 1; q < 16; q++) if (q * 8 < lim) r += vals[q];
            }
            double s1 = r + __shfl_down(r, 1, 64);
            double s2 = s1 + __shfl_down(s1, 2, 64);
            double s3 = s2 + __shfl_down(s2, 4, 64);
            if (l < nl && k == 0) {
                double res;
                if (n < 8) { res = 0.0; for (int i = 0; i < n; i++) res += elem(o + i); }
                else { res = s3; for (int i = lim; i < n; i++) res += elem(o + i); }
                leaf_sum[l] = res;
            }
        }
        __syncthreads();
        if (lane == 0) acc += combine_leaves(nl, leaf_sum, leaf_dep, st_v, st_a);
    }
    return acc;
}

__device__ __forceinline__ double diag_sum_sequential(const double* __restrict__ M2, int64_t ld2, const IndexMap& m, int n_used,
                                                      int off)
{
    __shared__ double seq_buf[1024];
    const int lane = threadIdx.x, len = n_used - off;
    double acc = 0.0;
    for (int c0 = 0; c0 < len; c0 += 1024) {
        const int cnt = len - c0 < 1024 ? len - c0 : 1024;
        __syncthreads();
        for (int e = lane; e < cnt; e += 64) seq_buf[e] = M2[(int64_t)m.at(c0 + e) * ld2 + m.at(c0 + e + off)];
        __syncthreads();
        if (lane == 0) acc = serial_sum_lds(seq_buf, 0, cnt, acc);
    }
    return acc;
}

static bool numba_trace_order()
{
    const char* v = getenv("HICMI_P2_TRACE_ORDER");
    return v && (v[0] == 'n' || v[0] == 'N') && (v[1] == 'u' || v[1] == 'U') && (v[2] == 'm' || v[2] == 'M') && (v[3] == 'b' || v[3] == 'B');
}

__global__ __launch_bounds__(64) void k_p2_diag_sums(const double* __restrict__ M2, int64_t ld2,
                                                     const int32_t* __restrict__ perms, int n_used,
                                                     double* __restrict__ T, int sequential)
{
    const int cand = blockIdx.y, off = diag_of_block(blockIdx.x);
    if (off >= n_used) return;
    const IndexMap m = {perms ? perms + (int64_t)cand * n_used : nullptr, kNoSplice, 0, 0, 0};
    const double acc = sequential ? diag_sum_sequential(M2, ld2, m, n_used, off) : diag_sum_body(M2, ld2, m, n_used, off);
    if (threadIdx.x == 0) T[(int64_t)cand * n_used + off] = acc;
}

static constexpr int SERIAL_LDS_MAX = 8192;

__global__ __launch_bounds__(256) void k_p2_total_exact(const double* __restrict__ T, int n_used, double* __restrict__ total)
{
    extern __shared__ __attribute__((aligned(16))) unsigned char smem_t[];
    double* t = reinterpret_cast<double*>(smem_t);
    const bool staged = n_used <= SERIAL_LDS_MAX;
    if (staged) {
        for (int i = threadIdx.x; i < n_used; i += 256) t[i] = T[i];
        __syncthreads();
    }
    if (threadIdx.x != 0) return;
    double acc = 0.0;
    if (staged) acc = serial_sum_lds(t, 1, n_used, 0.0);
    else {
        for (int i = 1; i < n_used; i++) acc += T[i];
    }
    total[0] = acc;
}

__device__ __forceinline__ void cost_exact_body(const double* __restrict__ tg, int n_used, double total,
                                                double* __restrict__ wg, double* __restrict__ score_out)
{
    extern __shared__ __attribute__((aligned(16))) unsigned char smem_c[];
    const bool staged = n_used <= SERIAL_LDS_MAX;
    double* w = staged ? reinterpret_cast<double*>(smem_c) : wg;
    if (staged) {
        for (int i = threadIdx.x; i < n_used; i += 256) w[i] = tg[i];
        __syncthreads();
    }
    if (threadIdx.x == 0) {
        double cum = 0.0;
        if (staged) serial_prefix_lds(w, 1, n_used, 0.0);
        else {
            for (int i = 1; i < n_used; i++) { cum += tg[i]; w[i] = cum; }
        }
    }
    __syncthreads();
    for (int i = 1 + threadIdx.x; i < n_used; i += 256) w[i] = w[i] / total / (double)i;
    __syncthreads();
    if (threadIdx.x == 0) {
        double cost = 0.0;
        if (staged) cost = serial_sum_lds(w, 1, n_used, 0.0);
        else for (int i = 1; i < n_used; i++) cost += w[i];
        score_out[0] = cost;
    }
}

__global__ __launch_bounds__(256) void k_p2_cost_exact(const double* __restrict__ T, int n_used, double total,
                                                       double* __restrict__ work, double* __restrict__ scores)
{
    const int cand = blockIdx.x;
    cost_exact_body(T + (int64_t)cand * n_used, n_used, total, work + (int64_t)cand * n_used, scores + cand);
}

static std::atomic<int> g_lds_total{0}, g_lds_cost{0}, g_lds_score{0}, g_lds_insb_cost{0};

static size_t serial_lds_bytes(int n) { return n <= SERIAL_LDS_MAX ? (((size_t)n * sizeof(double)) + 15) & ~(size_t)15 : 16; }

void launch_p2_total(const double* M2, int64_t ld2, int n, double* T, double* total, hipStream_t s)
{
    if (n > 1) hipLaunchKernelGGL(k_p2_diag_sums, dim3(diag_grid(n), 1), dim3(64), 0, s, M2, ld2, (const int32_t*)nullptr, n, T, 0);
    ensure_dynamic_lds(reinterpret_cast<const void*>(k_p2_total_exact), g_lds_total, 65536);
    hipLaunchKernelGGL(k_p2_total_exact, dim3(1), dim3(256), serial_lds_bytes(n), s, T, n, total);
}

void launch_p2_total_perm(const double* M2, int64_t ld2, const int32_t* d_perm, int n, double* T, double* total,
                          hipStream_t s)
{
    if (n > 1) hipLaunchKernelGGL(k_p2_diag_sums, dim3(diag_grid(n), 1), dim3(64), 0, s, M2, ld2, d_perm, n, T, 0);
    ensure_dynamic_lds(reinterpret_cast<const void*>(k_p2_total_exact), g_lds_total, 65536);
    hipLaunchKernelGGL(k_p2_total_exact, dim3(1), dim3(256), serial_lds_bytes(n), s, T, n, total);
}

void launch_p2_score_exact(const double* M2, int64_t ld2, const int32_t* perms, int n_cand, int n_used, double total,
                           double* T, double* work, double* scores, hipStream_t s)
{
    if (n_cand <= 0) return;
    if (n_used > 1) hipLaunchKernelGGL(k_p2_diag_sums, dim3(diag_grid(n_used), n_cand), dim3(64), 0, s, M2, ld2, perms, n_used, T,
                                       numba_trace_order() ? 1 : 0);
    ensure_dynamic_lds(reinterpret_cast<const void*>(k_p2_cost_exact), g_lds_cost, 65536);
    hipLaunchKernelGGL(k_p2_cost_exact, dim3(n_cand), dim3(256), serial_lds_bytes(n_used), s, T, n_used, total, work, scores);
}

__global__ __launch_bounds__(64) void k_insb_diag_cand(const InsStep* __restrict__ steps, int sequential)
{
    const InsStep& d = steps[blockIdx.y];
    if (!d.active || d.st->fail >= 0) return;
    const int ns = d.st->n_short;
    if (ns == 0) return;
    const int n_used = d.n_arr + d.L, off = diag_of_block(blockIdx.x);
    if (off >= n_used) return;
    {
        const IndexMap m = {d.pos_cur, d.n_arr, 0x3fffffff, d.new_start, 0};
        const double acc = diag_sum_body(d.M2, d.ld2, m, n_used, off);
        if (threadIdx.x == 0) d.T_total[off] = acc;
    }
    for (int q = 0; q < ns; q++) {
        const IndexMap m = {d.pos_cur, d.packed_cur[d.S + d.st->gap[q]], d.L, d.new_start, d.st->rev[q]};
        const double acc = sequential ? diag_sum_sequential(d.M2, d.ld2, m, n_used, off) : diag_sum_body(d.M2, d.ld2, m, n_used, off);
        if (threadIdx.x == 0) d.T_cand[(int64_t)q * n_used + off] = acc;
    }
}

__global__ __launch_bounds__(256) void k_insb_cost(const InsStep* __restrict__ steps)
{
    extern __shared__ __attribute__((aligned(16))) unsigned char smem_ic[];
    __shared__ double s_total;
    const InsStep& d = steps[blockIdx.y];
    if (!d.active || d.st->fail >= 0) return;
    const int cand = blockIdx.x;
    if (cand >= d.st->n_short) return;
    const int n_used = d.n_arr + d.L;
    {
        double* t = reinterpret_cast<double*>(smem_ic);
        const bool staged = n_used <= SERIAL_LDS_MAX;
        if (staged) {
            for (int i = threadIdx.x; i < n_used; i += 256) t[i] = d.T_total[i];
            __syncthreads();
        }
        if (threadIdx.x == 0) {
            double acc = 0.0;
            if (staged) acc = serial_sum_lds(t, 1, n_used, 0.0);
            else for (int i = 1; i < n_used; i++) acc += d.T_total[i];
            s_total = acc;
            if (cand == 0) d.st->total = acc;
        }
        __syncthreads();
    }
    cost_exact_body(d.T_cand + (int64_t)cand * n_used, n_used, s_total, d.work + (int64_t)cand * n_used, d.st->lit + cand);
}

void launch_insb_diag_cand(const InsStep* steps, int n_chrom, int max_n_used, hipStream_t s)
{
    if (max_n_used < 2) return;
    hipLaunchKernelGGL(k_insb_diag_cand, dim3(diag_grid(max_n_used), n_chrom), dim3(64), 0, s, steps, numba_trace_order() ? 1 : 0);
}

void launch_insb_cost(const InsStep* steps, int n_chrom, int max_n_used, hipStream_t s)
{
    ensure_dynamic_lds(reinterpret_cast<const void*>(k_insb_cost), g_lds_insb_cost, 65536);
    const int max_staged = max_n_used < SERIAL_LDS_MAX ? max_n_used : SERIAL_LDS_MAX;
    hipLaunchKernelGGL(k_insb_cost, dim3(INS_MAXC, n_chrom), dim3(256), serial_lds_bytes(max_staged), s, steps);
}

__global__ __launch_bounds__(256) void k_p2_score(const double* __restrict__ M2, int64_t ld2,
                                                  const int32_t* __restrict__ perms, int n_used,
                                                  const double* __restrict__ H, double total,
                                                  double* __restrict__ scores)
{
    extern __shared__ __attribute__((aligned(16))) unsigned char smem[];
    int32_t* p = reinterpret_cast<int32_t*>(smem);
    __shared__ double s_w[4];
    const int cand = blockIdx.x, tid = threadIdx.x, lane = tid & 63, wave = tid >> 6;
    const int32_t* __restrict__ src = perms + (int64_t)cand * n_used;
    for (int i = tid; i < n_used; i += 256) p[i] = src[i];
    __syncthreads();
    const double hn = H[n_used - 1];
    double acc = 0.0;
    for (int a = wave; a < n_used - 1; a += 4) {
        const double* __restrict__ row = M2 + (int64_t)p[a] * ld2;
        for (int b = a + 1 + lane; b < n_used; b += 64) acc += row[p[b]] * (hn - H[b - a - 1]);
    }
    acc = wave_sum(acc);
    if (lane == 0) s_w[wave] = acc;
    __syncthreads();
    if (tid == 0) scores[cand] = ((s_w[0] + s_w[1]) + (s_w[2] + s_w[3])) / total;
}

void launch_p2_score(const double* M2, int64_t ld2, const int32_t* perms, int n_cand, int n_used, const double* H,
                     double, double total, double* scores, hipStream_t s)
{
    if (n_cand <= 0) return;
    size_t lds = (((size_t)n_used * sizeof(int32_t)) + 15) & ~(size_t)15;
    ensure_dynamic_lds(reinterpret_cast<const void*>(k_p2_score), g_lds_score, lds);
    hipLaunchKernelGGL(k_p2_score, dim3(n_cand), dim3(256), lds, s, M2, ld2, perms, n_used, H, total, scores);
}

}
```

hic_genome_assembler_amd/csrc/k_part2_insert.hip:

```cpp
#include "hicmi_internal.h"

namespace hicmi {

__global__ void k_insb_reset(const InsStep* __restrict__ steps)
{
    InsState* st = steps[blockIdx.x].st;
    if (threadIdx.x == 0 && steps[blockIdx.x].active) { st->fail = -1; st->n_short = 0; st->direct = 0; }
}

void launch_insb_reset(const InsStep* steps, int n_chrom, hipStream_t s)
{
    hipLaunchKernelGGL(k_insb_reset, dim3(n_chrom), dim3(64), 0, s, steps);
}

static constexpr int SL_THREADS = 256;
static constexpr int SL_LIST = 64;
static constexpr int SL_STAGE_MAX = 8192;

__global__ __launch_bounds__(SL_THREADS) void k_insb_shortlist(const InsStep* __restrict__ steps, int n_base_blocks,
                                                               double near_top, int max_c)
{
    extern __shared__ __attribute__((aligned(16))) unsigned char smem_sl[];
    double* buf = reinterpret_cast<double*>(smem_sl);
    __shared__ double s_base, s_wmax[SL_THREADS / 64];
    __shared__ int s_any[SL_THREADS / 64], s_cnt, s_list[SL_LIST];
    const InsStep& d = steps[blockIdx.x];
    InsState* st = d.st;
    const int tid = threadIdx.x;
    if (!d.active || st->fail >= 0) return;
    const int S = d.S, n_arr = d.n_arr;
    const double* __restrict__ partial = d.partial;
    const int32_t* __restrict__ arr_pos = d.packed_cur + S;
    double* part = buf + S + 1;
    const bool staged = n_arr <= SL_STAGE_MAX;
    const int n_stage = n_base_blocks + (staged ? n_arr : 0);
    for (int i = tid; i < n_stage; i += SL_THREADS) part[i] = partial[i];
    if (tid == 0) s_cnt = 0;
    __syncthreads();
    for (int g = tid; g < S; g += SL_THREADS) {
        const int P0 = arr_pos[g], P1 = arr_pos[g + 1];
        double acc = 0.0;
        if (staged) for (int u = P0; u < P1; u++) acc += part[n_base_blocks + u];
        else for (int u = P0; u < P1; u++) acc += partial[n_base_blocks + u];
        buf[g + 1] = acc;
    }
    __syncthreads();
    if (tid == 0) {
        s_base = serial_sum_lds(part, 0, n_base_blocks, 0.0);
        buf[0] = 0.0;
        serial_prefix_lds(buf, 1, S + 1, 0.0);
    }
    __syncthreads();
    const double base = s_base;
    const double* __restrict__ cross = partial + n_base_blocks + n_arr;
    const int n_cand = 2 * (S + 1);
    auto fast_of = [&](int i) -> double {
        const int g = i >> 1, first = g & 1;
        const int r = (i & 1) ? (first ^ 1) : first;
        return base - buf[g] + cross[2 * g + r];
    };
    double mx = -__builtin_inf();
    int any = 0;
    for (int i = tid; i < n_cand; i += SL_THREADS) {
        const double v = fast_of(i);
        if (isfinite(v)) { any = 1; if (v > mx) mx = v; }
    }
#pragma unroll
    for (int off = 32; off >= 1; off >>= 1) {
        const double o = __shfl_xor(mx, off, 64);
        const int oa = __shfl_xor(any, off, 64);
        if (o > mx) mx = o;
        any |= oa;
    }
    if ((tid & 63) == 0) { s_wmax[tid >> 6] = mx; s_any[tid >> 6] = any; }
    __syncthreads();
    double top = 0.0;
    int have = 0;
    for (int w = 0; w < SL_THREADS / 64; w++) { if (s_wmax[w] > top) top = s_wmax[w]; have |= s_any[w]; }
    if (!have) {
        if (tid == 0) { st->n_short = 0; st->direct = 0; }
        return;
    }
    const double thr = top - fabs(top) * near_top;
    for (int i = tid; i < n_cand; i += SL_THREADS) {
        const double v = fast_of(i);
        if (isfinite(v) && v >= thr) {
            const int slot = atomicAdd(&s_cnt, 1);
            if (slot < SL_LIST) s_list[slot] = i;
        }
    }
    __syncthreads();
    if (tid == 0) {
        int cnt = s_cnt;
        st->direct = 0;
        if (cnt > max_c && !(d.L == 1 && cnt <= 2 * max_c && cnt <= SL_LIST)) { st->fail = d.step; st->n_short = 0; return; }
        for (int a = 1; a < cnt; a++) {
            const int v = s_list[a];
            int b = a - 1;
            while (b >= 0 && s_list[b] > v) { s_list[b + 1] = s_list[b]; b--; }
            s_list[b + 1] = v;
        }
        if (d.L == 1) {
            int w = 0;
            for (int q = 0; q < cnt; q++) {
                const int i = s_list[q];
                if ((i & 1) && w > 0 && s_list[w - 1] == i - 1) continue;
                s_list[w++] = i;
            }
            cnt = w;
            if (cnt > max_c) { st->fail = d.step; st->n_short = 0; return; }
        }
        for (int q = 0; q < cnt; q++) {
            const int i = s_list[q], g = i >> 1, first = g & 1;
            st->idx[q] = i; st->gap[q] = g; st->rev[q] = (i & 1) ? (first ^ 1) : first;
        }
        if (cnt == 1 && !d.last && top > 0.0) { st->direct = 1; st->n_short = 0; }
        else st->n_short = cnt;
    }
}

static std::atomic<int> g_lds_shortlist{0};

void launch_insb_shortlist(const InsStep* steps, int n_chrom, int max_S, int max_n_arr, int n_base_blocks, double near_top,
                           int max_c, hipStream_t s)
{
    const int need = (max_S + 1) + n_base_blocks + (max_n_arr < SL_STAGE_MAX ? max_n_arr : SL_STAGE_MAX);
    const size_t lds = (((size_t)need * sizeof(double)) + 15) & ~(size_t)15;
    ensure_dynamic_lds(reinterpret_cast<const void*>(k_insb_shortlist), g_lds_shortlist, lds);
    hipLaunchKernelGGL(k_insb_shortlist, dim3(n_chrom), dim3(SL_THREADS), lds, s, steps, n_base_blocks, near_top,
                       max_c < 1 ? 1 : (max_c > INS_MAXC ? INS_MAXC : max_c));
}

__global__ __launch_bounds__(256) void k_insb_apply(const InsStep* __restrict__ steps)
{
    const InsStep& d = steps[blockIdx.y];
    const InsState* __restrict__ st = d.st;
    if (!d.active || st->fail >= 0) return;
    const int n_arr = d.n_arr, S = d.S, L = d.L, n_new = n_arr + L;
    if ((int)blockIdx.x * 256 >= n_new && blockIdx.x != 0) return;
    double best = 0.0;
    int pick = -1;
    const int ns = st->n_short, direct = st->direct;
    for (int q = 0; q < ns; q++) if (st->lit[q] > best) { best = st->lit[q]; pick = q; }
    if (direct) { pick = 0; best = __builtin_nan(""); }
    const int gap = pick >= 0 ? st->gap[pick] : 0, rev = pick >= 0 ? st->rev[pick] : 0;
    const int32_t* __restrict__ id_in = d.packed_cur;
    const int32_t* __restrict__ pos_in = d.packed_cur + S;
    const int32_t* __restrict__ rev_in = d.packed_cur + 2 * S + 1;
    const int P = pos_in[gap];
    const int pos = blockIdx.x * 256 + threadIdx.x;
    if (pos < n_new) {
        int v;
        if (pos < P) v = d.pos_cur[pos];
        else if (pos < P + L) v = d.new_start + (rev ? L - 1 - (pos - P) : pos - P);
        else v = d.pos_cur[pos - L];
        d.pos_nxt[pos] = v;
    }
    if (blockIdx.x == 0) {
        const int S1 = S + 1;
        int32_t* __restrict__ id_out = d.packed_nxt;
        int32_t* __restrict__ pos_out = d.packed_nxt + S1;
        int32_t* __restrict__ rev_out = d.packed_nxt + 2 * S1 + 1;
        for (int j = threadIdx.x; j < S1; j += 256) {
            id_out[j] = j < gap ? id_in[j] : (j == gap ? d.new_id : id_in[j - 1]);
            rev_out[j] = j < gap ? rev_in[j] : (j == gap ? rev : rev_in[j - 1]);
        }
        for (int j = threadIdx.x; j <= S1; j += 256) pos_out[j] = j <= gap ? pos_in[j] : pos_in[j - 1] + L;
        if (threadIdx.x == 0) { d.log->gap = gap; d.log->rev = rev; d.log->best = pick >= 0 ? best : 0.0; d.log->n_short = direct ? -1 : ns; }
    }
}

void launch_insb_apply(const InsStep* steps, int n_chrom, int max_n_used, hipStream_t s)
{
    hipLaunchKernelGGL(k_insb_apply, dim3((max_n_used + 255) / 256, n_chrom), dim3(256), 0, s, steps);
}

}
```

hic_genome_assembler_amd/csrc/k_part2_search.hip:

```cpp
#include "hicmi_internal.h"

namespace hicmi {

__device__ __forceinline__ double block_sum_1024(double v, double* s_w)
{
    v = wave_sum_s(v);
    if ((threadIdx.x & 63) == 0) s_w[threadIdx.x >> 6] = v;
    __syncthreads();
    double acc = 0.0;
#pragma unroll
    for (int i = 0; i < 16; i++) acc += s_w[i];
    return acc;
}

static size_t perm_lds_bytes(int n) { return (((size_t)n * sizeof(int32_t)) + 15) & ~(size_t)15; }

__global__ __launch_bounds__(256) void k_arr_materialize(const int32_t* __restrict__ packed, int S,
                                                         const int32_t* __restrict__ scaf_start,
                                                         const int32_t* __restrict__ scaf_len, int n_arr,
                                                         int32_t* __restrict__ pos2sel)
{
    const int32_t* __restrict__ arr_id = packed;
    const int32_t* __restrict__ arr_pos = packed + S;
    const int32_t* __restrict__ arr_rev = packed + 2 * S + 1;
    int q = blockIdx.x * 256 + threadIdx.x;
    if (q >= n_arr) return;
    int lo = 0, hi = S;
    while (hi - lo > 1) {
        int mid = (lo + hi) >> 1;
        if (arr_pos[mid] <= q) lo = mid; else hi = mid;
    }
    int sc = arr_id[lo], off = q - arr_pos[lo], len = scaf_len[sc];
    pos2sel[q] = scaf_start[sc] + (arr_rev[lo] ? len - 1 - off : off);
}

void launch_arr_materialize(const int32_t* packed, int S, const int32_t* scaf_start, const int32_t* scaf_len, int n_arr,
                            int32_t* pos2sel, hipStream_t s)
{
    if (n_arr <= 0) return;
    hipLaunchKernelGGL(k_arr_materialize, dim3((n_arr + 255) / 256), dim3(256), 0, s, packed, S, scaf_start, scaf_len,
                       n_arr, pos2sel);
}

__global__ __launch_bounds__(256) void k_p2_base_partial(const double* __restrict__ M2, int64_t ld2,
                                                         const int32_t* __restrict__ pos2sel, int n_arr,
                                                         const double* __restrict__ H, int n_tot,
                                                         double* __restrict__ partial)
{
    extern __shared__ __attribute__((aligned(16))) unsigned char smem[];
    int32_t* p = reinterpret_cast<int32_t*>(smem);
    for (int q = threadIdx.x; q < n_arr; q += 256) p[q] = pos2sel[q];
    __syncthreads();
    base_partial_body(M2, ld2, p, n_arr, H, n_tot, blockIdx.x, gridDim.x, partial + blockIdx.x);
}

static std::atomic<int> g_lds_base{0}, g_lds_straddle{0}, g_lds_cross{0}, g_lds_wdelta{0}, g_lds_wdelta1{0}, g_lds_wdelta_blk{0}, g_lds_wG{0}, g_lds_insb_base{0}, g_lds_insb_fast{0};

void launch_p2_base_partial(const double* M2, int64_t ld2, const int32_t* pos2sel, int n_arr, const double* H, int n_tot,
                            int n_blocks, double* out, hipStream_t s)
{
    ensure_dynamic_lds(reinterpret_cast<const void*>(k_p2_base_partial), g_lds_base, perm_lds_bytes(n_arr));
    hipLaunchKernelGGL(k_p2_base_partial, dim3(n_blocks), dim3(256), perm_lds_bytes(n_arr), s, M2, ld2, pos2sel, n_arr, H,
                       n_tot, out);
}

__device__ __forceinline__ void straddle_body(const double* __restrict__ M2, int64_t ld2, const int32_t* p, int n_arr,
                                              const int32_t* __restrict__ arr_pos, int g, int L,
                                              const double* __restrict__ H, double* s_w, double* __restrict__ out)
{
    const int lane = threadIdx.x & 63, wave = threadIdx.x >> 6;
    const int P0 = arr_pos[g], P1 = arr_pos[g + 1];
    const int len = P1 - P0, n_out = n_arr - len;
    double acc = 0.0;
    for (int u = P0 + wave; u < P1; u += 16) {
        const double* __restrict__ row = M2 + (int64_t)p[u] * ld2;
#pragma unroll 8
        for (int qq = lane; qq < n_out; qq += 64) {
            const bool before = qq < P0;
            const int pos = before ? qq : qq + len;
            const int d = before ? u - pos : pos - u;
            const double w = H[d + L - 1] - H[d - 1];
            const double v = row[p[pos]] * w;
            acc += before ? -v : v;
        }
    }
    double sum = block_sum_1024(acc, s_w);
    if (threadIdx.x == 0) out[0] = sum;
}

__device__ __forceinline__ void cross_body(const double* __restrict__ M2, int64_t ld2, const int32_t* p, int n_arr,
                                           const int32_t* __restrict__ arr_pos, int g, int r, int new_start, int L,
                                           const double* __restrict__ H, double* s_w, double* __restrict__ out)
{
    const int lane = threadIdx.x & 63, wave = threadIdx.x >> 6;
    const int P = arr_pos[g];
    const double hn = H[n_arr + L - 1];
    double acc = 0.0;
    for (int e = wave; e < L; e += 16) {
        const int xe = new_start + (r ? L - 1 - e : e);
        const double* __restrict__ row = M2 + (int64_t)xe * ld2;
#pragma unroll 4
        for (int q = lane; q < n_arr; q += 64) {
            int d = q < P ? (P + e - q) : (q + L - (P + e));
            acc += row[p[q]] * (hn - H[d - 1]);
        }
        for (int e2 = e + 1 + lane; e2 < L; e2 += 64) {
            int x2 = new_start + (r ? L - 1 - e2 : e2);
            acc += row[x2] * (hn - H[e2 - e - 1]);
        }
    }
    double sum = block_sum_1024(acc, s_w);
    if (threadIdx.x == 0) out[0] = sum;
}

__global__ __launch_bounds__(1024) void k_p2_insert_straddle(const double* __restrict__ M2, int64_t ld2,
                                                            const int32_t* __restrict__ pos2sel, int n_arr,
                                                            const int32_t* __restrict__ arr_pos, int L,
                                                            const double* __restrict__ H, double* __restrict__ D)
{
    extern __shared__ __attribute__((aligned(16))) unsigned char smem[];
    int32_t* p = reinterpret_cast<int32_t*>(smem);
    __shared__ double s_w[16];
    for (int q = threadIdx.x; q < n_arr; q += 1024) p[q] = pos2sel[q];
    __syncthreads();
    straddle_body(M2, ld2, p, n_arr, arr_pos, blockIdx.x, L, H, s_w, D + blockIdx.x);
}

__global__ __launch_bounds__(1024) void k_p2_insert_cross(const double* __restrict__ M2, int64_t ld2,
                                                         const int32_t* __restrict__ pos2sel, int n_arr,
                                                         const int32_t* __restrict__ arr_pos, int new_start, int L,
                                                         const double* __restrict__ H, double* __restrict__ cross)
{
    extern __shared__ __attribute__((aligned(16))) unsigned char smem[];
    int32_t* p = reinterpret_cast<int32_t*>(smem);
    __shared__ double s_w[16];
    for (int q = threadIdx.x; q < n_arr; q += 1024) p[q] = pos2sel[q];
    __syncthreads();
    cross_body(M2, ld2, p, n_arr, arr_pos, blockIdx.x >> 1, blockIdx.x & 1, new_start, L, H, s_w, cross + blockIdx.x);
}

void launch_p2_insert_delta(const double* M2, int64_t ld2, const int32_t* pos2sel, int n_arr, const int32_t* arr_pos,
                            int S, int new_start, int L, const double* H, int n_base_blocks, double* out, hipStream_t s)
{
    const size_t lds = perm_lds_bytes(n_arr);
    launch_p2_base_partial(M2, ld2, pos2sel, n_arr, H, n_arr + L, n_base_blocks, out, s);
    ensure_dynamic_lds(reinterpret_cast<const void*>(k_p2_insert_straddle), g_lds_straddle, lds);
    ensure_dynamic_lds(reinterpret_cast<const void*>(k_p2_insert_cross), g_lds_cross, lds);
    hipLaunchKernelGGL(k_p2_insert_straddle, dim3(S), dim3(1024), lds, s, M2, ld2, pos2sel, n_arr, arr_pos, L, H,
                       out + n_base_blocks);
    hipLaunchKernelGGL(k_p2_insert_cross, dim3(2 * (S + 1)), dim3(1024), lds, s, M2, ld2, pos2sel, n_arr, arr_pos, new_start,
                       L, H, out + n_base_blocks + S);
}

__global__ __launch_bounds__(256) void k_insb_base(const InsStep* __restrict__ steps, int n_base_blocks)
{
    extern __shared__ __attribute__((aligned(16))) unsigned char smem[];
    int32_t* p = reinterpret_cast<int32_t*>(smem);
    const InsStep& d = steps[blockIdx.y];
    if (!d.active || d.st->fail >= 0) return;
    for (int q = threadIdx.x; q < d.n_arr; q += 256) p[q] = d.pos_cur[q];
    __syncthreads();
    base_partial_body(d.M2, d.ld2, p, d.n_arr, d.H, d.n_arr + d.L, blockIdx.x, n_base_blocks, d.partial + blockIdx.x);
}

__global__ __launch_bounds__(256) void k_insb_fast(const InsStep* __restrict__ steps, int n_base_blocks, int n_row_blocks,
                                                   int n_cross_blocks)
{
    extern __shared__ __attribute__((aligned(16))) unsigned char smem[];
    __shared__ double s_w[4];
    const InsStep& d = steps[blockIdx.y];
    if (!d.active || d.st->fail >= 0) return;
    const int S = d.S, n_arr = d.n_arr, L = d.L;
    const int lane = threadIdx.x & 63, wave = threadIdx.x >> 6;
    const int32_t* __restrict__ p = d.pos_cur;
    const int32_t* __restrict__ arr_pos = d.packed_cur + S;
    const double* __restrict__ H = d.H;
    const int n_base_here = (int)gridDim.x - n_row_blocks - n_cross_blocks;
    const int bx = (int)blockIdx.x - n_base_here;
    if (bx < 0) {
        const int slab = blockIdx.x;
        int32_t* pl = reinterpret_cast<int32_t*>(smem);
        for (int q = threadIdx.x; q < n_arr; q += 256) pl[q] = p[q];
        __syncthreads();
        base_partial_body(d.M2, d.ld2, pl, n_arr, H, n_arr + L, slab, n_base_blocks, d.partial + slab);
        return;
    }
    if (bx < n_row_blocks) {
        const int u = bx * 4 + wave;
        if (u >= n_arr) return;
        int below = 0;
        for (int j = lane; j <= S; j += 64) below += arr_pos[j] <= u;
#pragma unroll
        for (int off = 32; off >= 1; off >>= 1) below += __shfl_xor(below, off, 64);
        const int g = below - 1;
        const int P0 = arr_pos[g], P1 = arr_pos[g + 1];
        const double* __restrict__ row = d.M2 + (int64_t)p[u] * d.ld2;
        double acc = 0.0;
#pragma unroll 4
        for (int pos = lane; pos < P0; pos += 64) {
            const int dd = u - pos;
            acc -= row[p[pos]] * (H[dd + L - 1] - H[dd - 1]);
        }
#pragma unroll 4
        for (int pos = P1 + lane; pos < n_arr; pos += 64) {
            const int dd = pos - u;
            acc += row[p[pos]] * (H[dd + L - 1] - H[dd - 1]);
        }
        acc = wave_sum_s(acc);
        if (lane == 0) d.partial[n_base_blocks + u] = acc;
        return;
    }
    const int c = bx - n_row_blocks;
    if (c >= 2 * (S + 1)) return;
    const int g = c >> 1, r = c & 1, P = arr_pos[g];
    const double hn = H[n_arr + L - 1];
    double acc = 0.0;
    for (int e = wave; e < L; e += 4) {
        const int xe = d.new_start + (r ? L - 1 - e : e);
        const double* __restrict__ row = d.M2 + (int64_t)xe * d.ld2;
#pragma unroll 4
        for (int q = lane; q < n_arr; q += 64) {
            const int dd = q < P ? (P + e - q) : (q + L - (P + e));
            acc += row[p[q]] * (hn - H[dd - 1]);
        }
        for (int e2 = e + 1 + lane; e2 < L; e2 += 64) {
            const int x2 = d.new_start + (r ? L - 1 - e2 : e2);
            acc += row[x2] * (hn - H[e2 - e - 1]);
        }
    }
    const double sum = block_sum_256(acc, s_w);
    if (threadIdx.x == 0) d.partial[n_base_blocks + n_arr + c] = sum;
}

void launch_insb_fast(const InsStep* steps, int n_chrom, int max_S, int max_n_arr, int n_base_blocks, hipStream_t s)
{
    const size_t lds = perm_lds_bytes(max_n_arr);
    const int n_row_blocks = (max_n_arr + 3) / 4, n_cross_blocks = 2 * (max_S + 1);
    static const bool split = getenv("HICMI_P2_INSB_SPLIT") != nullptr;
    if (split) {
        ensure_dynamic_lds(reinterpret_cast<const void*>(k_insb_base), g_lds_insb_base, lds);
        hipLaunchKernelGGL(k_insb_base, dim3(n_base_blocks, n_chrom), dim3(256), lds, s, steps, n_base_blocks);
    }
    ensure_dynamic_lds(reinterpret_cast<const void*>(k_insb_fast), g_lds_insb_fast, lds);
    hipLaunchKernelGGL(k_insb_fast, dim3(n_row_blocks + n_cross_blocks + (split ? 0 : n_base_blocks), n_chrom), dim3(256), lds, s,
                       steps, n_base_blocks, n_row_blocks, n_cross_blocks);
}

static constexpr int G_TILE = 2048;
static constexpr int G_TMAX = 8;

template <bool H_IN_LDS>
__global__ __launch_bounds__(256) void k_p2_window_G(const double* __restrict__ M2, int64_t ld2,
                                                     const int32_t* __restrict__ pos2sel, int n,
                                                     const WindowBatchEntry* __restrict__ wb,
                                                     const double* H, double* __restrict__ G_all)
{
    extern __shared__ __attribute__((aligned(16))) unsigned char smem_g[];
    __shared__ double vals[G_TILE];
    __shared__ double part[4][64];
    const WindowBatchEntry& we = wb[blockIdx.y];
    const int p0 = we.p0, m = we.m;
    const int x = blockIdx.x, tid = threadIdx.x, tl = tid & 63, seg = tid >> 6;
    if (x >= m) return;
    double* __restrict__ G = G_all + we.g_off;
    const double* __restrict__ row = M2 + (int64_t)pos2sel[p0 + x] * ld2;
    const double hn = H[n - 1];
    if (H_IN_LDS) {
        double* hl = reinterpret_cast<double*>(smem_g);
        for (int i = tid; i < n; i += 256) hl[i] = H[i];
        __syncthreads();
        H = hl;
    }
    const int n_out = n - m;
    for (int tbase = 0; tbase < m; tbase += 64 * G_TMAX) {
        double acc[G_TMAX];
#pragma unroll
        for (int i = 0; i < G_TMAX; i++) acc[i] = 0.0;
        for (int base = 0; base < n_out; base += G_TILE) {
            const int cnt = n_out - base < G_TILE ? n_out - base : G_TILE;
            __syncthreads();
            for (int e = tid; e < cnt; e += 256) {
                int qq = base + e;
                vals[e] = row[pos2sel[qq < p0 ? qq : qq + m]];
            }
            __syncthreads();
            const int e0 = (cnt * seg) >> 2, e1 = (cnt * (seg + 1)) >> 2;
#pragma unroll
            for (int i = 0; i < G_TMAX; i++) {
                const int t = tbase + i * 64 + tl;
                if (t < m) {
                    const int pt = p0 + t;
                    double a = acc[i];
                    for (int e = e0; e < e1; e++) {
                        int qq = base + e;
                        int d = qq < p0 ? pt - qq : qq + m - pt;
                        a += vals[e] * (hn - H[d - 1]);
                    }
                    acc[i] = a;
                }
            }
        }
#pragma unroll
        for (int i = 0; i < G_TMAX; i++) {
            __syncthreads();
            part[seg][tl] = acc[i];
            __syncthreads();
            const int t = tbase + i * 64 + tl;
            if (seg == 0 && t < m) G[(int64_t)x * m + t] = (part[0][tl] + part[1][tl]) + (part[2][tl] + part[3][tl]);
        }
    }
}

static constexpr int WD_PER_WAVE = 4;
template <int WD_WAVES, bool BLOCK_IN_LDS>
__global__ __launch_bounds__(WD_WAVES * 64) void k_p2_window_delta(const double* __restrict__ M2, int64_t ld2, int n, int k,
                                                         const WindowBatchEntry* __restrict__ wb,
                                                         const int8_t* __restrict__ orders,
                                                         const uint8_t* __restrict__ orients, int n_ori, int n_cand,
                                                         const double* __restrict__ H, const double* __restrict__ G_all,
                                                         double* __restrict__ delta_all,
                                                         const int32_t* __restrict__ pos2sel, int max_m)
{
    extern __shared__ __attribute__((aligned(16))) unsigned char smem[];
    __shared__ int s_start[8], s_len[8], s_off[8], s_rev[8];
    __shared__ int s_ord[WD_WAVES][8], s_ori[WD_WAVES][8], s_slot[WD_WAVES][9];
    const WindowBatchEntry& we = wb[blockIdx.y];
    const int m = we.m;
    const double* __restrict__ G = G_all + we.g_off;
    const int tid = threadIdx.x, lane = tid & 63, wave = tid >> 6;
    int32_t* useq = reinterpret_cast<int32_t*>(smem) + (int64_t)wave * 2 * m;
    int32_t* xseq = useq + m;
    double* wt = reinterpret_cast<double*>(smem + (((size_t)max_m * 2 * WD_WAVES * sizeof(int32_t) + 15) & ~(size_t)15));
    double* wblk = wt + max_m;
    if (tid < k) {
        s_start[tid] = we.w.start[tid]; s_len[tid] = we.w.len[tid]; s_off[tid] = we.w.off[tid]; s_rev[tid] = we.w.rev[tid];
    }
    if (BLOCK_IN_LDS) {
        const int32_t* __restrict__ wsel = pos2sel + we.p0;
        for (int e = tid; e < m * m; e += WD_WAVES * 64) {
            const int x = e / m, y = e - x * m;
            wblk[e] = M2[(int64_t)wsel[x] * ld2 + wsel[y]];
        }
    }
    const double hn = H[n - 1];
    for (int d = tid; d < m; d += WD_WAVES * 64) wt[d] = d ? hn - H[d - 1] : 0.0;
    const int mm = m * m, ds = 64 / m, dt = 64 - ds * m;
    for (int it = 0; it < WD_PER_WAVE; it++) {
        const int c = (blockIdx.x * WD_WAVES + wave) * WD_PER_WAVE + it;
        const bool live = c < n_cand;
        if (live && lane < k) {
            s_ord[wave][lane] = orders[(int64_t)(c / n_ori) * k + lane];
            s_ori[wave][lane] = orients[(int64_t)(c % n_ori) * k + lane];
        }
        __syncthreads();
        if (live && lane == 0) {
            int acc_len = 0;
            s_slot[wave][0] = 0;
            for (int j = 0; j < k; j++) { acc_len += s_len[s_ord[wave][j]]; s_slot[wave][j + 1] = acc_len; }
        }
        __syncthreads();
        if (live) {
            for (int t = lane; t < m; t += 64) {
                int j = 0;
                while (j + 1 < k && s_slot[wave][j + 1] <= t) j++;
                const int jj = s_ord[wave][j], len = s_len[jj];
                const int ep = t - s_slot[wave][j];
                const int e = s_ori[wave][j] ? len - 1 - ep : ep;
                useq[t] = s_start[jj] + e;
                xseq[t] = s_off[jj] + (s_rev[jj] ? len - 1 - e : e);
            }
        }
        __syncthreads();
        if (live) {
            double acc = 0.0;
            for (int t = lane; t < m; t += 64) acc += G[(int64_t)xseq[t] * m + t];
            int ps = lane / m, pt = lane - ps * m;
#pragma unroll 8
            for (int q = lane; q < mm; q += 64) {
                const double v = BLOCK_IN_LDS ? wblk[xseq[ps] * m + xseq[pt]] : M2[(int64_t)useq[ps] * ld2 + useq[pt]];
                acc += v * wt[pt > ps ? pt - ps : 0];
                const int npt = pt + dt;
                const bool carry = npt >= m;
                ps += ds + (carry ? 1 : 0);
                pt = carry ? npt - m : npt;
            }
            acc = wave_sum_s(acc);
            if (lane == 0) delta_all[(int64_t)blockIdx.y * n_cand + c] = acc;
        }
        __syncthreads();
    }
}

void launch_p2_window_batch_G(const double* M2, int64_t ld2, const int32_t* pos2sel, int n, const WindowBatchEntry* wb, int n_win,
                              int max_m, const double* H, double* G_all, hipStream_t s)
{
    if (n_win <= 0 || max_m <= 0) return;
    const size_t h_lds = (((size_t)n * sizeof(double)) + 15) & ~(size_t)15;
    if (h_lds <= 96 * 1024) {
        ensure_dynamic_lds(reinterpret_cast<const void*>(k_p2_window_G<true>), g_lds_wG, h_lds);
        hipLaunchKernelGGL(k_p2_window_G<true>, dim3(max_m, n_win), dim3(256), h_lds, s, M2, ld2, pos2sel, n, wb, H, G_all);
    } else {
        hipLaunchKernelGGL(k_p2_window_G<false>, dim3(max_m, n_win), dim3(256), 0, s, M2, ld2, pos2sel, n, wb, H, G_all);
    }
}

void launch_p2_window_batch_delta(const double* M2, int64_t ld2, const int32_t* pos2sel, int n, int k,
                                  const WindowBatchEntry* wb, int n_win, int max_m, const int8_t* orders, const uint8_t* orients,
                                  int n_ord, int n_ori, const double* H, const double* G_all, double* delta_all, hipStream_t s)
{
    if (n_win <= 0 || max_m <= 0) return;
    const int n_cand = n_ord * n_ori;
    const size_t wt_bytes = (size_t)max_m * sizeof(double);
    const size_t seq4 = ((((size_t)max_m * 2 * 4 * sizeof(int32_t)) + 15) & ~(size_t)15) + wt_bytes;
    if (max_m <= 128) {
        const size_t lds = seq4 + (size_t)max_m * max_m * sizeof(double);
        ensure_dynamic_lds(reinterpret_cast<const void*>(k_p2_window_delta<4, true>), g_lds_wdelta_blk, lds);
        hipLaunchKernelGGL((k_p2_window_delta<4, true>), dim3((n_cand + 4 * WD_PER_WAVE - 1) / (4 * WD_PER_WAVE), n_win), dim3(256),
                           lds, s, M2, ld2, n, k, wb, orders, orients, n_ori, n_cand, H, G_all, delta_all, pos2sel, max_m);
    } else if (max_m <= 4096) {
        ensure_dynamic_lds(reinterpret_cast<const void*>(k_p2_window_delta<4, false>), g_lds_wdelta, seq4);
        hipLaunchKernelGGL((k_p2_window_delta<4, false>), dim3((n_cand + 4 * WD_PER_WAVE - 1) / (4 * WD_PER_WAVE), n_win), dim3(256),
                           seq4, s, M2, ld2, n, k, wb, orders, orients, n_ori, n_cand, H, G_all, delta_all, pos2sel, max_m);
    } else {
        const size_t lds = ((((size_t)max_m * 2 * sizeof(int32_t)) + 15) & ~(size_t)15) + wt_bytes;
        ensure_dynamic_lds(reinterpret_cast<const void*>(k_p2_window_delta<1, false>), g_lds_wdelta1, lds);
        hipLaunchKernelGGL((k_p2_window_delta<1, false>), dim3((n_cand + WD_PER_WAVE - 1) / WD_PER_WAVE, n_win), dim3(64), lds, s, M2,
                           ld2, n, k, wb, orders, orients, n_ori, n_cand, H, G_all, delta_all, pos2sel, max_m);
    }
}

}
```

Measured before the change: 124,400.

## Fuse insertion shortlist and apply into fast/cost kernels via last-block tickets

Adds per-step atomic ticket counters so the last workgroup finishing the insb_fast pass runs the shortlist selection inline, and the last block of the cost pass runs the apply step, removing two kernel launches per insertion step. Partial results are published with agent-scope atomic stores and the last block acquires before reading them. In exchange it adds memsets of the ticket and state buffers, extra LDS that may reduce occupancy, and serial tail work done by a single workgroup.

```diff
diff --git a/hic_genome_assembler_amd/csrc/api.hip b/hic_genome_assembler_amd/csrc/api.hip
--- a/hic_genome_assembler_amd/csrc/api.hip
+++ b/hic_genome_assembler_amd/csrc/api.hip
@@ -146,6 +146,7 @@
     DevBuf<double> d_ins_partial;
     DevBuf<unsigned char> d_ins_blob;
     DevBuf<InsStep> d_ins_steps;
+    DevBuf<uint32_t> d_ins_tick;
     DevBuf<SupRec> d_sup_recs;
     DevBuf<BrkRec> d_brk_recs;
     DevBuf<InvRec> d_inv_recs;
@@ -3404,6 +3405,8 @@
     if (nj == 0) return HICMI_OK;
     const int NB = kBaseSlabs;
     static const int max_c = getenv("HICMI_P2_INS_MAXC") ? atoi(getenv("HICMI_P2_INS_MAXC")) : INS_MAXC;
+    static const bool tails = !getenv("HICMI_P2_INSB_UNFUSED") && !getenv("HICMI_P2_INSB_SPLIT");
+    static const int count_off = getenv("HICMI_TEST_INSB_COUNT_OFF") ? 1 : 0;
     int64_t steps_max = 0;
     std::vector<size_t> blob_off((size_t)nj);
     size_t blob_bytes = 0;
@@ -3435,6 +3438,7 @@
     std::vector<InsStep> table((size_t)(steps_max * nj));
     std::vector<int> max_n_used((size_t)steps_max, 0), max_S((size_t)steps_max, 0), max_n_arr((size_t)steps_max, 0);
     double algo = 0.0;
+    int64_t n_tick = 0;
     for (int j = 0; j < nj; j++) {
         InsJob& job = *jobs[(size_t)j];
         hicmi_ctx* c = job.c;
@@ -3458,6 +3462,8 @@
             d.pos_cur = pos2sel[cur]; d.pos_nxt = pos2sel[nxt]; d.packed_cur = packed[cur]; d.packed_nxt = packed[nxt];
             d.T_total = c->d_ins_T; d.T_cand = c->d_ins_T + n_max; d.work = c->d_ins_T + (1 + (int64_t)INS_MAXC) * n_max;
             d.partial = c->d_ins_partial; d.log = log + t;
+            d.tick = reinterpret_cast<uint32_t*>(n_tick * sizeof(uint32_t));
+            n_tick += ins_tick_words(NB + (n_arr + 3) / 4 + 2 * (job.S + t + 1) + count_off);
             d.n_arr = (int32_t)n_arr; d.S = (int32_t)(job.S + t); d.L = L; d.new_start = c->h_scaf_start[(size_t)nid];
             d.new_id = nid; d.active = 1; d.step = (int32_t)t; d.last = t == n_steps - 1;
             max_n_used[(size_t)t] = std::max(max_n_used[(size_t)t], (int)(n_arr + L));
@@ -3468,19 +3474,25 @@
             n_arr += L;
         }
     }
+    rc = ensure(lead->d_ins_tick, n_tick);
+    if (rc) return rc;
+    for (InsStep& d : table)
+        if (d.active) d.tick = lead->d_ins_tick + reinterpret_cast<uintptr_t>(d.tick) / sizeof(uint32_t);
     rc = upload(lead, lead->d_ins_steps, table.data(), sizeof(InsStep) * table.size());
     if (rc) return rc;
     {
         Timed timed(lead, F_P2_INSERT, algo);
+        HIPCHK(hipMemsetAsync(lead->d_ins_blob, 0xff, blob_bytes, lead->stream));
+        HIPCHK(hipMemsetAsync(lead->d_ins_tick, 0, sizeof(uint32_t) * (size_t)n_tick, lead->stream));
         launch_insb_reset(lead->d_ins_steps, nj, lead->stream);
         for (int64_t t = 0; t < steps_max; t++) {
             const InsStep* st_t = lead->d_ins_steps + t * nj;
             const int nu = max_n_used[(size_t)t];
-            launch_insb_fast(st_t, nj, max_S[(size_t)t], max_n_arr[(size_t)t], NB, lead->stream);
-            launch_insb_shortlist(st_t, nj, max_S[(size_t)t], max_n_arr[(size_t)t], NB, kNearTop, max_c, lead->stream);
+            launch_insb_fast(st_t, nj, max_S[(size_t)t], max_n_arr[(size_t)t], NB, tails, kNearTop, max_c, count_off, lead->stream);
+            if (!tails) launch_insb_shortlist(st_t, nj, max_S[(size_t)t], max_n_arr[(size_t)t], NB, kNearTop, max_c, lead->stream);
             launch_insb_diag_cand(st_t, nj, nu, lead->stream);
-            launch_insb_cost(st_t, nj, nu, lead->stream);
-            launch_insb_apply(st_t, nj, nu, lead->stream);
+            launch_insb_cost(st_t, nj, nu, tails, count_off, lead->stream);
+            if (!tails) launch_insb_apply(st_t, nj, nu, lead->stream);
         }
     }
     HIPCHK(hipGetLastError());
diff --git a/hic_genome_assembler_amd/csrc/hicmi_internal.h b/hic_genome_assembler_amd/csrc/hicmi_internal.h
--- a/hic_genome_assembler_amd/csrc/hicmi_internal.h
+++ b/hic_genome_assembler_amd/csrc/hicmi_internal.h
@@ -277,9 +277,8 @@
     return (s_w[0] + s_w[1]) + (s_w[2] + s_w[3]);
 }
 
-__device__ __forceinline__ void base_partial_body(const double* __restrict__ M2, int64_t ld2, const int32_t* p, int n_arr,
-                                                  const double* __restrict__ H, int n_tot, int blk, int n_blk,
-                                                  double* __restrict__ out)
+__device__ __forceinline__ double base_partial_sum(const double* __restrict__ M2, int64_t ld2, const int32_t* p, int n_arr,
+                                                   const double* __restrict__ H, int n_tot, int blk, int n_blk)
 {
     __shared__ double s_w[4];
     const int lane = threadIdx.x & 63, wave = threadIdx.x >> 6;
@@ -290,7 +289,14 @@
 #pragma unroll 4
         for (int b = a + 1 + lane; b < n_arr; b += 64) acc += row[p[b]] * (hn - H[b - a - 1]);
     }
-    double sum = block_sum_256(acc, s_w);
+    return block_sum_256(acc, s_w);
+}
+
+__device__ __forceinline__ void base_partial_body(const double* __restrict__ M2, int64_t ld2, const int32_t* p, int n_arr,
+                                                  const double* __restrict__ H, int n_tot, int blk, int n_blk,
+                                                  double* __restrict__ out)
+{
+    const double sum = base_partial_sum(M2, ld2, p, n_arr, H, n_tot, blk, n_blk);
     if (threadIdx.x == 0) out[0] = sum;
 }
 
@@ -335,10 +341,16 @@
 }
 
 static constexpr int INS_MAXC = 8;
+static constexpr int INS_TICK_LINE = 32, INS_TICK_GROUP = 64;
+inline int64_t ins_tick_words(int64_t fast_tickets)
+{
+    return INS_TICK_LINE * (2 + (fast_tickets + INS_TICK_GROUP - 1) / INS_TICK_GROUP);
+}
 struct InsState {
     int32_t fail;
     int32_t n_short;
-    int32_t direct, pad;
+    int32_t direct;
+    int32_t done;
     int32_t gap[INS_MAXC], rev[INS_MAXC], idx[INS_MAXC];
     double total;
     double lit[INS_MAXC];
@@ -350,14 +362,16 @@
     const int32_t* packed_cur; int32_t* packed_nxt;
     double *T_total, *T_cand, *work, *partial;
     InsState* st; InsLog* log;
+    uint32_t* tick;
     int32_t n_arr, S, L, new_start, new_id, active, step, last;
 };
 void launch_insb_reset(const InsStep* steps, int n_chrom, hipStream_t s);
-void launch_insb_fast(const InsStep* steps, int n_chrom, int max_S, int max_n_arr, int n_base_blocks, hipStream_t s);
+void launch_insb_fast(const InsStep* steps, int n_chrom, int max_S, int max_n_arr, int n_base_blocks, bool tail, double near_top,
+                      int max_c, int count_off, hipStream_t s);
 void launch_insb_shortlist(const InsStep* steps, int n_chrom, int max_S, int max_n_arr, int n_base_blocks, double near_top,
                            int max_c, hipStream_t s);
 void launch_insb_diag_cand(const InsStep* steps, int n_chrom, int max_n_used, hipStream_t s);
-void launch_insb_cost(const InsStep* steps, int n_chrom, int max_n_used, hipStream_t s);
+void launch_insb_cost(const InsStep* steps, int n_chrom, int max_n_used, bool tail, int count_off, hipStream_t s);
 void launch_insb_apply(const InsStep* steps, int n_chrom, int max_n_used, hipStream_t s);
 
 static constexpr int SUP_BASE_SLABS = 64;
diff --git a/hic_genome_assembler_amd/csrc/insb_tail.h b/hic_genome_assembler_amd/csrc/insb_tail.h
--- /dev/null
+++ b/hic_genome_assembler_amd/csrc/insb_tail.h
@@ -0,0 +1,199 @@
+#pragma once
+#include "hicmi_internal.h"
+
+namespace hicmi {
+
+static constexpr int SL_THREADS = 256;
+static constexpr int SL_LIST = 64;
+static constexpr int SL_STAGE_MAX = 8192;
+
+inline int insb_clamp_max_c(int max_c) { return max_c < 1 ? 1 : (max_c > INS_MAXC ? INS_MAXC : max_c); }
+
+typedef __attribute__((address_space(1))) double insb_gf64;
+typedef __attribute__((address_space(1))) uint32_t insb_gu32;
+
+__device__ __forceinline__ void publish_f64(double* p, double v)
+{
+    __hip_atomic_store((insb_gf64*)p, v, __ATOMIC_RELAXED, __HIP_MEMORY_SCOPE_AGENT);
+}
+
+__device__ __forceinline__ bool draw_last_ticket(uint32_t* top, uint32_t* sub, int k, int expect, int* s_last)
+{
+    asm volatile("s_waitcnt vmcnt(0)" ::: "memory");
+    __syncthreads();
+    if (threadIdx.x == 0) {
+        const int grp = k / INS_TICK_GROUP, n_grp = (expect + INS_TICK_GROUP - 1) / INS_TICK_GROUP;
+        const int left = expect - grp * INS_TICK_GROUP, members = left < INS_TICK_GROUP ? left : INS_TICK_GROUP;
+        int last = 1;
+        if (n_grp > 1) {
+            const uint32_t t = __hip_atomic_fetch_add((insb_gu32*)(sub + grp * INS_TICK_LINE), 1u, __ATOMIC_RELAXED, __HIP_MEMORY_SCOPE_AGENT);
+            last = t == (uint32_t)(members - 1);
+        }
+        if (last) {
+            const uint32_t t = __hip_atomic_fetch_add((insb_gu32*)top, 1u, __ATOMIC_RELAXED, __HIP_MEMORY_SCOPE_AGENT);
+            last = t == (uint32_t)((n_grp > 1 ? n_grp : expect) - 1);
+        }
+        if (last) {
+            __builtin_amdgcn_fence(__ATOMIC_ACQUIRE, "agent");
+            asm volatile("s_waitcnt vmcnt(0)" ::: "memory");
+        }
+        *s_last = last;
+    }
+    __syncthreads();
+    return *s_last != 0;
+}
+
+__device__ __forceinline__ int32_t wg_load(const int32_t* p) { return __hip_atomic_load(p, __ATOMIC_RELAXED, __HIP_MEMORY_SCOPE_WORKGROUP); }
+__device__ __forceinline__ double wg_load(const double* p) { return __hip_atomic_load(p, __ATOMIC_RELAXED, __HIP_MEMORY_SCOPE_WORKGROUP); }
+
+__device__ __forceinline__ int insb_shortlist_body(const InsStep& d, InsState* st, double* buf, int lds_doubles,
+                                                   int n_base_blocks, double near_top, int max_c)
+{
+    __shared__ double s_base, s_wmax[SL_THREADS / 64];
+    __shared__ int s_any[SL_THREADS / 64], s_cnt, s_list[SL_LIST];
+    const int tid = threadIdx.x;
+    const int S = d.S, n_arr = d.n_arr;
+    const double* partial = d.partial;
+    const int32_t* __restrict__ arr_pos = d.packed_cur + S;
+    double* part = buf + S + 1;
+    const bool staged = n_arr <= SL_STAGE_MAX && (S + 1) + n_base_blocks + n_arr <= lds_doubles;
+    const int n_stage = n_base_blocks + (staged ? n_arr : 0);
+    for (int i0 = tid; i0 < n_stage; i0 += 8 * SL_THREADS) {
+        double v[8];
+#pragma unroll
+        for (int q = 0; q < 8; q++) v[q] = i0 + q * SL_THREADS < n_stage ? partial[i0 + q * SL_THREADS] : 0.0;
+#pragma unroll
+        for (int q = 0; q < 8; q++) if (i0 + q * SL_THREADS < n_stage) part[i0 + q * SL_THREADS] = v[q];
+    }
+    if (tid == 0) s_cnt = 0;
+    __syncthreads();
+    for (int g = tid; g < S; g += SL_THREADS) {
+        const int P0 = arr_pos[g], P1 = arr_pos[g + 1];
+        double acc = 0.0;
+        if (staged) for (int u = P0; u < P1; u++) acc += part[n_base_blocks + u];
+        else for (int u = P0; u < P1; u++) acc += partial[n_base_blocks + u];
+        buf[g + 1] = acc;
+    }
+    __syncthreads();
+    if (tid == 0) {
+        s_base = serial_sum_lds(part, 0, n_base_blocks, 0.0);
+        buf[0] = 0.0;
+        serial_prefix_lds(buf, 1, S + 1, 0.0);
+    }
+    __syncthreads();
+    const double base = s_base;
+    const double* cross = partial + n_base_blocks + n_arr;
+    const int n_cand = 2 * (S + 1);
+    auto fast_of = [&](int i) -> double {
+        const int g = i >> 1, first = g & 1;
+        const int r = (i & 1) ? (first ^ 1) : first;
+        return base - buf[g] + cross[2 * g + r];
+    };
+    double mx = -__builtin_inf();
+    int any = 0;
+    for (int i = tid; i < n_cand; i += SL_THREADS) {
+        const double v = fast_of(i);
+        if (isfinite(v)) { any = 1; if (v > mx) mx = v; }
+    }
+#pragma unroll
+    for (int off = 32; off >= 1; off >>= 1) {
+        const double o = __shfl_xor(mx, off, 64);
+        const int oa = __shfl_xor(any, off, 64);
+        if (o > mx) mx = o;
+        any |= oa;
+    }
+    if ((tid & 63) == 0) { s_wmax[tid >> 6] = mx; s_any[tid >> 6] = any; }
+    __syncthreads();
+    double top = 0.0;
+    int have = 0;
+    for (int w = 0; w < SL_THREADS / 64; w++) { if (s_wmax[w] > top) top = s_wmax[w]; have |= s_any[w]; }
+    if (!have) {
+        if (tid == 0) { st->n_short = 0; st->direct = 0; }
+        return 1;
+    }
+    const double thr = top - fabs(top) * near_top;
+    for (int i = tid; i < n_cand; i += SL_THREADS) {
+        const double v = fast_of(i);
+        if (isfinite(v) && v >= thr) {
+            const int slot = atomicAdd(&s_cnt, 1);
+            if (slot < SL_LIST) s_list[slot] = i;
+        }
+    }
+    __syncthreads();
+    if (tid == 0) {
+        int cnt = s_cnt;
+        st->direct = 0;
+        if (cnt > max_c && !(d.L == 1 && cnt <= 2 * max_c && cnt <= SL_LIST)) { st->fail = d.step; st->n_short = 0; return 0; }
+        for (int a = 1; a < cnt; a++) {
+            const int v = s_list[a];
+            int b = a - 1;
+            while (b >= 0 && s_list[b] > v) { s_list[b + 1] = s_list[b]; b--; }
+            s_list[b + 1] = v;
+        }
+        if (d.L == 1) {
+            int w = 0;
+            for (int q = 0; q < cnt; q++) {
+                const int i = s_list[q];
+                if ((i & 1) && w > 0 && s_list[w - 1] == i - 1) continue;
+                s_list[w++] = i;
+            }
+            cnt = w;
+            if (cnt > max_c) { st->fail = d.step; st->n_short = 0; return 0; }
+        }
+        for (int q = 0; q < cnt; q++) {
+            const int i = s_list[q], g = i >> 1, first = g & 1;
+            st->idx[q] = i; st->gap[q] = g; st->rev[q] = (i & 1) ? (first ^ 1) : first;
+        }
+        if (cnt == 1 && !d.last && top > 0.0) { st->direct = 1; st->n_short = 0; return 1; }
+        st->n_short = cnt;
+        return cnt == 0;
+    }
+    return 0;
+}
+
+__device__ __forceinline__ void insb_apply_body(const InsStep& d, InsState* st, int bx)
+{
+    const int n_arr = d.n_arr, S = d.S, L = d.L, n_new = n_arr + L;
+    if (bx * 256 >= n_new && bx != 0) return;
+    double best = 0.0;
+    int pick = -1;
+    const int ns = wg_load(&st->n_short), direct = wg_load(&st->direct);
+    for (int q = 0; q < ns; q++) { const double v = wg_load(&st->lit[q]); if (v > best) { best = v; pick = q; } }
+    if (direct) { pick = 0; best = __builtin_nan(""); }
+    const int gap = pick >= 0 ? wg_load(&st->gap[pick]) : 0, rev = pick >= 0 ? wg_load(&st->rev[pick]) : 0;
+    const int32_t* __restrict__ id_in = d.packed_cur;
+    const int32_t* __restrict__ pos_in = d.packed_cur + S;
+    const int32_t* __restrict__ rev_in = d.packed_cur + 2 * S + 1;
+    const int P = pos_in[gap];
+    const int pos = bx * 256 + threadIdx.x;
+    if (pos < n_new) {
+        int v;
+        if (pos < P) v = d.pos_cur[pos];
+        else if (pos < P + L) v = d.new_start + (rev ? L - 1 - (pos - P) : pos - P);
+        else v = d.pos_cur[pos - L];
+        d.pos_nxt[pos] = v;
+    }
+    if (bx == 0) {
+        const int S1 = S + 1;
+        int32_t* __restrict__ id_out = d.packed_nxt;
+        int32_t* __restrict__ pos_out = d.packed_nxt + S1;
+        int32_t* __restrict__ rev_out = d.packed_nxt + 2 * S1 + 1;
+        for (int j = threadIdx.x; j < S1; j += 256) {
+            id_out[j] = j < gap ? id_in[j] : (j == gap ? d.new_id : id_in[j - 1]);
+            rev_out[j] = j < gap ? rev_in[j] : (j == gap ? rev : rev_in[j - 1]);
+        }
+        for (int j = threadIdx.x; j <= S1; j += 256) pos_out[j] = j <= gap ? pos_in[j] : pos_in[j - 1] + L;
+        if (threadIdx.x == 0) {
+            d.log->gap = gap; d.log->rev = rev; d.log->best = pick >= 0 ? best : 0.0; d.log->n_short = direct ? -1 : ns;
+            st->done = d.step + 1;
+        }
+    }
+}
+
+__device__ __forceinline__ void insb_apply_all(const InsStep& d, InsState* st)
+{
+    const int n_new = d.n_arr + d.L;
+    for (int bx = 0; bx == 0 || bx * 256 < n_new; bx++) insb_apply_body(d, st, bx);
+}
+
+}
diff --git a/hic_genome_assembler_amd/csrc/k_part2.hip b/hic_genome_assembler_amd/csrc/k_part2.hip
--- a/hic_genome_assembler_amd/csrc/k_part2.hip
+++ b/hic_genome_assembler_amd/csrc/k_part2.hip
@@ -1,6 +1,7 @@
 #include <cstdlib>
 
 #include "hicmi_internal.h"
+#include "insb_tail.h"
 
 namespace hicmi {
 
@@ -149,8 +150,8 @@
     total[0] = acc;
 }
 
-__device__ __forceinline__ void cost_exact_body(const double* __restrict__ tg, int n_used, double total,
-                                                double* __restrict__ wg, double* __restrict__ score_out)
+__device__ __forceinline__ double cost_exact_value(const double* __restrict__ tg, int n_used, double total,
+                                                   double* __restrict__ wg)
 {
     extern __shared__ __attribute__((aligned(16))) unsigned char smem_c[];
     const bool staged = n_used <= SERIAL_LDS_MAX;
@@ -169,12 +170,19 @@
     __syncthreads();
     for (int i = 1 + threadIdx.x; i < n_used; i += 256) w[i] = w[i] / total / (double)i;
     __syncthreads();
+    double cost = 0.0;
     if (threadIdx.x == 0) {
-        double cost = 0.0;
         if (staged) cost = serial_sum_lds(w, 1, n_used, 0.0);
         else for (int i = 1; i < n_used; i++) cost += w[i];
-        score_out[0] = cost;
-    }
+    }
+    return cost;
+}
+
+__device__ __forceinline__ void cost_exact_body(const double* __restrict__ tg, int n_used, double total,
+                                                double* __restrict__ wg, double* __restrict__ score_out)
+{
+    const double cost = cost_exact_value(tg, n_used, total, wg);
+    if (threadIdx.x == 0) score_out[0] = cost;
 }
 
 __global__ __launch_bounds__(256) void k_p2_cost_exact(const double* __restrict__ T, int n_used, double total,
@@ -184,7 +192,7 @@
     cost_exact_body(T + (int64_t)cand * n_used, n_used, total, work + (int64_t)cand * n_used, scores + cand);
 }
 
-static std::atomic<int> g_lds_total{0}, g_lds_cost{0}, g_lds_score{0}, g_lds_insb_cost{0};
+static std::atomic<int> g_lds_total{0}, g_lds_cost{0}, g_lds_score{0}, g_lds_insb_cost{0}, g_lds_insb_cost_unfused{0};
 
 static size_t serial_lds_bytes(int n) { return n <= SERIAL_LDS_MAX ? (((size_t)n * sizeof(double)) + 15) & ~(size_t)15 : 16; }
 
@@ -216,7 +224,7 @@
 __global__ __launch_bounds__(64) void k_insb_diag_cand(const InsStep* __restrict__ steps, int sequential)
 {
     const InsStep& d = steps[blockIdx.y];
-    if (!d.active || d.st->fail >= 0) return;
+    if (!d.active || d.st->fail >= 0 || d.st->done != d.step) return;
     const int ns = d.st->n_short;
     if (ns == 0) return;
     const int n_used = d.n_arr + d.L, off = diag_of_block(blockIdx.x);
@@ -233,14 +241,14 @@
     }
 }
 
-__global__ __launch_bounds__(256) void k_insb_cost(const InsStep* __restrict__ steps)
-{
-    extern __shared__ __attribute__((aligned(16))) unsigned char smem_ic[];
+template <bool TAIL>
+__device__ __forceinline__ void insb_cost_pass(const InsStep& d, unsigned char* smem_ic, int count_off)
+{
     __shared__ double s_total;
-    const InsStep& d = steps[blockIdx.y];
-    if (!d.active || d.st->fail >= 0) return;
-    const int cand = blockIdx.x;
-    if (cand >= d.st->n_short) return;
+    __shared__ int s_last;
+    if (!d.active || d.st->fail >= 0 || d.st->done != d.step) return;
+    const int cand = blockIdx.x, ns = d.st->n_short;
+    if (cand >= ns) return;
     const int n_used = d.n_arr + d.L;
     {
         double* t = reinterpret_cast<double*>(smem_ic);
@@ -258,7 +266,26 @@
         }
         __syncthreads();
     }
-    cost_exact_body(d.T_cand + (int64_t)cand * n_used, n_used, s_total, d.work + (int64_t)cand * n_used, d.st->lit + cand);
+    const double cost = cost_exact_value(d.T_cand + (int64_t)cand * n_used, n_used, s_total, d.work + (int64_t)cand * n_used);
+    if (threadIdx.x == 0) {
+        if (TAIL) publish_f64(d.st->lit + cand, cost);
+        else d.st->lit[cand] = cost;
+    }
+    if (!TAIL) return;
+    if (!draw_last_ticket(d.tick + INS_TICK_LINE, nullptr, cand, ns + count_off, &s_last)) return;
+    insb_apply_all(d, d.st);
+}
+
+__global__ __launch_bounds__(256) void k_insb_cost(const InsStep* __restrict__ steps, int count_off)
+{
+    extern __shared__ __attribute__((aligned(16))) unsigned char smem_ic[];
+    insb_cost_pass<true>(steps[blockIdx.y], smem_ic, count_off);
+}
+
+__global__ __launch_bounds__(256) void k_insb_cost_unfused(const InsStep* __restrict__ steps)
+{
+    extern __shared__ __attribute__((aligned(16))) unsigned char smem_ic[];
+    insb_cost_pass<false>(steps[blockIdx.y], smem_ic, 0);
 }
 
 void launch_insb_diag_cand(const InsStep* steps, int n_chrom, int max_n_used, hipStream_t s)
@@ -267,11 +294,13 @@
     hipLaunchKernelGGL(k_insb_diag_cand, dim3(diag_grid(max_n_used), n_chrom), dim3(64), 0, s, steps, numba_trace_order() ? 1 : 0);
 }
 
-void launch_insb_cost(const InsStep* steps, int n_chrom, int max_n_used, hipStream_t s)
+void launch_insb_cost(const InsStep* steps, int n_chrom, int max_n_used, bool tail, int count_off, hipStream_t s)
 {
     ensure_dynamic_lds(reinterpret_cast<const void*>(k_insb_cost), g_lds_insb_cost, 65536);
+    ensure_dynamic_lds(reinterpret_cast<const void*>(k_insb_cost_unfused), g_lds_insb_cost_unfused, 65536);
     const int max_staged = max_n_used < SERIAL_LDS_MAX ? max_n_used : SERIAL_LDS_MAX;
-    hipLaunchKernelGGL(k_insb_cost, dim3(INS_MAXC, n_chrom), dim3(256), serial_lds_bytes(max_staged), s, steps);
+    if (tail) hipLaunchKernelGGL(k_insb_cost, dim3(INS_MAXC, n_chrom), dim3(256), serial_lds_bytes(max_staged), s, steps, count_off);
+    else hipLaunchKernelGGL(k_insb_cost_unfused, dim3(INS_MAXC, n_chrom), dim3(256), serial_lds_bytes(max_staged), s, steps);
 }
 
 __global__ __launch_bounds__(256) void k_p2_score(const double* __restrict__ M2, int64_t ld2,
diff --git a/hic_genome_assembler_amd/csrc/k_part2_insert.hip b/hic_genome_assembler_amd/csrc/k_part2_insert.hip
--- a/hic_genome_assembler_amd/csrc/k_part2_insert.hip
+++ b/hic_genome_assembler_amd/csrc/k_part2_insert.hip
@@ -1,11 +1,12 @@
 #include "hicmi_internal.h"
+#include "insb_tail.h"
 
 namespace hicmi {
 
 __global__ void k_insb_reset(const InsStep* __restrict__ steps)
 {
     InsState* st = steps[blockIdx.x].st;
-    if (threadIdx.x == 0 && steps[blockIdx.x].active) { st->fail = -1; st->n_short = 0; st->direct = 0; }
+    if (threadIdx.x == 0 && steps[blockIdx.x].active) { st->fail = -1; st->n_short = 0; st->direct = 0; st->done = 0; }
 }
 
 void launch_insb_reset(const InsStep* steps, int n_chrom, hipStream_t s)
@@ -13,110 +14,14 @@
     hipLaunchKernelGGL(k_insb_reset, dim3(n_chrom), dim3(64), 0, s, steps);
 }
 
-static constexpr int SL_THREADS = 256;
-static constexpr int SL_LIST = 64;
-static constexpr int SL_STAGE_MAX = 8192;
-
 __global__ __launch_bounds__(SL_THREADS) void k_insb_shortlist(const InsStep* __restrict__ steps, int n_base_blocks,
-                                                               double near_top, int max_c)
+                                                               double near_top, int max_c, int lds_doubles)
 {
     extern __shared__ __attribute__((aligned(16))) unsigned char smem_sl[];
-    double* buf = reinterpret_cast<double*>(smem_sl);
-    __shared__ double s_base, s_wmax[SL_THREADS / 64];
-    __shared__ int s_any[SL_THREADS / 64], s_cnt, s_list[SL_LIST];
     const InsStep& d = steps[blockIdx.x];
     InsState* st = d.st;
-    const int tid = threadIdx.x;
-    if (!d.active || st->fail >= 0) return;
-    const int S = d.S, n_arr = d.n_arr;
-    const double* __restrict__ partial = d.partial;
-    const int32_t* __restrict__ arr_pos = d.packed_cur + S;
-    double* part = buf + S + 1;
-    const bool staged = n_arr <= SL_STAGE_MAX;
-    const int n_stage = n_base_blocks + (staged ? n_arr : 0);
-    for (int i = tid; i < n_stage; i += SL_THREADS) part[i] = partial[i];
-    if (tid == 0) s_cnt = 0;
-    __syncthreads();
-    for (int g = tid; g < S; g += SL_THREADS) {
-        const int P0 = arr_pos[g], P1 = arr_pos[g + 1];
-        double acc = 0.0;
-        if (staged) for (int u = P0; u < P1; u++) acc += part[n_base_blocks + u];
-        else for (int u = P0; u < P1; u++) acc += partial[n_base_blocks + u];
-        buf[g + 1] = acc;
-    }
-    __syncthreads();
-    if (tid == 0) {
-        s_base = serial_sum_lds(part, 0, n_base_blocks, 0.0);
-        buf[0] = 0.0;
-        serial_prefix_lds(buf, 1, S + 1, 0.0);
-    }
-    __syncthreads();
-    const double base = s_base;
-    const double* __restrict__ cross = partial + n_base_blocks + n_arr;
-    const int n_cand = 2 * (S + 1);
-    auto fast_of = [&](int i) -> double {
-        const int g = i >> 1, first = g & 1;
-        const int r = (i & 1) ? (first ^ 1) : first;
-        return base - buf[g] + cross[2 * g + r];
-    };
-    double mx = -__builtin_inf();
-    int any = 0;
-    for (int i = tid; i < n_cand; i += SL_THREADS) {
-        const double v = fast_of(i);
-        if (isfinite(v)) { any = 1; if (v > mx) mx = v; }
-    }
-#pragma unroll
-    for (int off = 32; off >= 1; off >>= 1) {
-        const double o = __shfl_xor(mx, off, 64);
-        const int oa = __shfl_xor(any, off, 64);
-        if (o > mx) mx = o;
-        any |= oa;
-    }
-    if ((tid & 63) == 0) { s_wmax[tid >> 6] = mx; s_any[tid >> 6] = any; }
-    __syncthreads();
-    double top = 0.0;
-    int have = 0;
-    for (int w = 0; w < SL_THREADS / 64; w++) { if (s_wmax[w] > top) top = s_wmax[w]; have |= s_any[w]; }
-    if (!have) {
-        if (tid == 0) { st->n_short = 0; st->direct = 0; }
-        return;
-    }
-    const double thr = top - fabs(top) * near_top;
-    for (int i = tid; i < n_cand; i += SL_THREADS) {
-        const double v = fast_of(i);
-        if (isfinite(v) && v >= thr) {
-            const int slot = atomicAdd(&s_cnt, 1);
-            if (slot < SL_LIST) s_list[slot] = i;
-        }
-    }
-    __syncthreads();
-    if (tid == 0) {
-        int cnt = s_cnt;
-        st->direct = 0;
-        if (cnt > max_c && !(d.L == 1 && cnt <= 2 * max_c && cnt <= SL_LIST)) { st->fail = d.step; st->n_short = 0; return; }
-        for (int a = 1; a < cnt; a++) {
-            const int v = s_list[a];
-            int b = a - 1;
-            while (b >= 0 && s_list[b] > v) { s_list[b + 1] = s_list[b]; b--; }
-            s_list[b + 1] = v;
-        }
-        if (d.L == 1) {
-            int w = 0;
-            for (int q = 0; q < cnt; q++) {
-                const int i = s_list[q];
-                if ((i & 1) && w > 0 && s_list[w - 1] == i - 1) continue;
-                s_list[w++] = i;
-            }
-            cnt = w;
-            if (cnt > max_c) { st->fail = d.step; st->n_short = 0; return; }
-        }
-        for (int q = 0; q < cnt; q++) {
-            const int i = s_list[q], g = i >> 1, first = g & 1;
-            st->idx[q] = i; st->gap[q] = g; st->rev[q] = (i & 1) ? (first ^ 1) : first;
-        }
-        if (cnt == 1 && !d.last && top > 0.0) { st->direct = 1; st->n_short = 0; }
-        else st->n_short = cnt;
-    }
+    if (!d.active || st->fail >= 0 || st->done != d.step) return;
+    insb_shortlist_body(d, st, reinterpret_cast<double*>(smem_sl), lds_doubles, n_base_blocks, near_top, max_c);
 }
 
 static std::atomic<int> g_lds_shortlist{0};
@@ -128,46 +33,14 @@
     const size_t lds = (((size_t)need * sizeof(double)) + 15) & ~(size_t)15;
     ensure_dynamic_lds(reinterpret_cast<const void*>(k_insb_shortlist), g_lds_shortlist, lds);
     hipLaunchKernelGGL(k_insb_shortlist, dim3(n_chrom), dim3(SL_THREADS), lds, s, steps, n_base_blocks, near_top,
-                       max_c < 1 ? 1 : (max_c > INS_MAXC ? INS_MAXC : max_c));
+                       insb_clamp_max_c(max_c), (int)(lds / sizeof(double)));
 }
 
 __global__ __launch_bounds__(256) void k_insb_apply(const InsStep* __restrict__ steps)
 {
     const InsStep& d = steps[blockIdx.y];
-    const InsState* __restrict__ st = d.st;
-    if (!d.active || st->fail >= 0) return;
-    const int n_arr = d.n_arr, S = d.S, L = d.L, n_new = n_arr + L;
-    if ((int)blockIdx.x * 256 >= n_new && blockIdx.x != 0) return;
-    double best = 0.0;
-    int pick = -1;
-    const int ns = st->n_short, direct = st->direct;
-    for (int q = 0; q < ns; q++) if (st->lit[q] > best) { best = st->lit[q]; pick = q; }
-    if (direct) { pick = 0; best = __builtin_nan(""); }
-    const int gap = pick >= 0 ? st->gap[pick] : 0, rev = pick >= 0 ? st->rev[pick] : 0;
-    const int32_t* __restrict__ id_in = d.packed_cur;
-    const int32_t* __restrict__ pos_in = d.packed_cur + S;
-    const int32_t* __restrict__ rev_in = d.packed_cur + 2 * S + 1;
-    const int P = pos_in[gap];
-    const int pos = blockIdx.x * 256 + threadIdx.x;
-    if (pos < n_new) {
-        int v;
-        if (pos < P) v = d.pos_cur[pos];
-        else if (pos < P + L) v = d.new_start + (rev ? L - 1 - (pos - P) : pos - P);
-        else v = d.pos_cur[pos - L];
-        d.pos_nxt[pos] = v;
-    }
-    if (blockIdx.x == 0) {
-        const int S1 = S + 1;
-        int32_t* __restrict__ id_out = d.packed_nxt;
-        int32_t* __restrict__ pos_out = d.packed_nxt + S1;
-        int32_t* __restrict__ rev_out = d.packed_nxt + 2 * S1 + 1;
-        for (int j = threadIdx.x; j < S1; j += 256) {
-            id_out[j] = j < gap ? id_in[j] : (j == gap ? d.new_id : id_in[j - 1]);
-            rev_out[j] = j < gap ? rev_in[j] : (j == gap ? rev : rev_in[j - 1]);
-        }
-        for (int j = threadIdx.x; j <= S1; j += 256) pos_out[j] = j <= gap ? pos_in[j] : pos_in[j - 1] + L;
-        if (threadIdx.x == 0) { d.log->gap = gap; d.log->rev = rev; d.log->best = pick >= 0 ? best : 0.0; d.log->n_short = direct ? -1 : ns; }
-    }
+    if (!d.active || d.st->fail >= 0) return;
+    insb_apply_body(d, d.st, (int)blockIdx.x);
 }
 
 void launch_insb_apply(const InsStep* steps, int n_chrom, int max_n_used, hipStream_t s)
diff --git a/hic_genome_assembler_amd/csrc/k_part2_search.hip b/hic_genome_assembler_amd/csrc/k_part2_search.hip
--- a/hic_genome_assembler_amd/csrc/k_part2_search.hip
+++ b/hic_genome_assembler_amd/csrc/k_part2_search.hip
@@ -1,4 +1,7 @@
+#include <cstdio>
+
 #include "hicmi_internal.h"
+#include "insb_tail.h"
 
 namespace hicmi {
 
@@ -54,7 +57,7 @@
     base_partial_body(M2, ld2, p, n_arr, H, n_tot, blockIdx.x, gridDim.x, partial + blockIdx.x);
 }
 
-static std::atomic<int> g_lds_base{0}, g_lds_straddle{0}, g_lds_cross{0}, g_lds_wdelta{0}, g_lds_wdelta1{0}, g_lds_wdelta_blk{0}, g_lds_wG{0}, g_lds_insb_base{0}, g_lds_insb_fast{0};
+static std::atomic<int> g_lds_base{0}, g_lds_straddle{0}, g_lds_cross{0}, g_lds_wdelta{0}, g_lds_wdelta1{0}, g_lds_wdelta_blk{0}, g_lds_wG{0}, g_lds_insb_base{0}, g_lds_insb_fast{0}, g_lds_insb_fast_unfused{0};
 
 void launch_p2_base_partial(const double* M2, int64_t ld2, const int32_t* pos2sel, int n_arr, const double* H, int n_tot,
                             int n_blocks, double* out, hipStream_t s)
@@ -157,19 +160,19 @@
     extern __shared__ __attribute__((aligned(16))) unsigned char smem[];
     int32_t* p = reinterpret_cast<int32_t*>(smem);
     const InsStep& d = steps[blockIdx.y];
-    if (!d.active || d.st->fail >= 0) return;
+    if (!d.active || d.st->fail >= 0 || d.st->done != d.step) return;
     for (int q = threadIdx.x; q < d.n_arr; q += 256) p[q] = d.pos_cur[q];
     __syncthreads();
     base_partial_body(d.M2, d.ld2, p, d.n_arr, d.H, d.n_arr + d.L, blockIdx.x, n_base_blocks, d.partial + blockIdx.x);
 }
 
-__global__ __launch_bounds__(256) void k_insb_fast(const InsStep* __restrict__ steps, int n_base_blocks, int n_row_blocks,
-                                                   int n_cross_blocks)
-{
-    extern __shared__ __attribute__((aligned(16))) unsigned char smem[];
+template <bool TAIL>
+__device__ __forceinline__ void insb_fast_pass(const InsStep& d, unsigned char* smem, int n_base_blocks, int n_row_blocks,
+                                               int n_cross_blocks, double near_top, int max_c, int count_off, int lds_doubles)
+{
     __shared__ double s_w[4];
-    const InsStep& d = steps[blockIdx.y];
-    if (!d.active || d.st->fail >= 0) return;
+    __shared__ int s_last;
+    if (!d.active || d.st->fail >= 0 || d.st->done != d.step) return;
     const int S = d.S, n_arr = d.n_arr, L = d.L;
     const int lane = threadIdx.x & 63, wave = threadIdx.x >> 6;
     const int32_t* __restrict__ p = d.pos_cur;
@@ -177,73 +180,131 @@
     const double* __restrict__ H = d.H;
     const int n_base_here = (int)gridDim.x - n_row_blocks - n_cross_blocks;
     const int bx = (int)blockIdx.x - n_base_here;
+    auto put = [](double* at, double v) { if (TAIL) publish_f64(at, v); else at[0] = v; };
     if (bx < 0) {
         const int slab = blockIdx.x;
         int32_t* pl = reinterpret_cast<int32_t*>(smem);
         for (int q = threadIdx.x; q < n_arr; q += 256) pl[q] = p[q];
         __syncthreads();
-        base_partial_body(d.M2, d.ld2, pl, n_arr, H, n_arr + L, slab, n_base_blocks, d.partial + slab);
-        return;
-    }
-    if (bx < n_row_blocks) {
+        const double sum = base_partial_sum(d.M2, d.ld2, pl, n_arr, H, n_arr + L, slab, n_base_blocks);
+        if (threadIdx.x == 0) put(d.partial + slab, sum);
+    } else if (bx < n_row_blocks) {
+        if (bx * 4 >= n_arr) return;
         const int u = bx * 4 + wave;
-        if (u >= n_arr) return;
-        int below = 0;
-        for (int j = lane; j <= S; j += 64) below += arr_pos[j] <= u;
+        if (u < n_arr) {
+            int below = 0;
+            for (int j = lane; j <= S; j += 64) below += arr_pos[j] <= u;
 #pragma unroll
-        for (int off = 32; off >= 1; off >>= 1) below += __shfl_xor(below, off, 64);
-        const int g = below - 1;
-        const int P0 = arr_pos[g], P1 = arr_pos[g + 1];
-        const double* __restrict__ row = d.M2 + (int64_t)p[u] * d.ld2;
+            for (int off = 32; off >= 1; off >>= 1) below += __shfl_xor(below, off, 64);
+            const int g = below - 1;
+            const int P0 = arr_pos[g], P1 = arr_pos[g + 1];
+            const double* __restrict__ row = d.M2 + (int64_t)p[u] * d.ld2;
+            double acc = 0.0;
+#pragma unroll 4
+            for (int pos = lane; pos < P0; pos += 64) {
+                const int dd = u - pos;
+                acc -= row[p[pos]] * (H[dd + L - 1] - H[dd - 1]);
+            }
+#pragma unroll 4
+            for (int pos = P1 + lane; pos < n_arr; pos += 64) {
+                const int dd = pos - u;
+                acc += row[p[pos]] * (H[dd + L - 1] - H[dd - 1]);
+            }
+            acc = wave_sum_s(acc);
+            if (lane == 0) put(d.partial + n_base_blocks + u, acc);
+        }
+    } else {
+        const int c = bx - n_row_blocks;
+        if (c >= 2 * (S + 1)) return;
+        const int g = c >> 1, r = c & 1, P = arr_pos[g];
+        const double hn = H[n_arr + L - 1];
         double acc = 0.0;
+        for (int e = wave; e < L; e += 4) {
+            const int xe = d.new_start + (r ? L - 1 - e : e);
+            const double* __restrict__ row = d.M2 + (int64_t)xe * d.ld2;
 #pragma unroll 4
-        for (int pos = lane; pos < P0; pos += 64) {
-            const int dd = u - pos;
-            acc -= row[p[pos]] * (H[dd + L - 1] - H[dd - 1]);
-        }
-#pragma unroll 4
-        for (int pos = P1 + lane; pos < n_arr; pos += 64) {
-            const int dd = pos - u;
-            acc += row[p[pos]] * (H[dd + L - 1] - H[dd - 1]);
-        }
-        acc = wave_sum_s(acc);
-        if (lane == 0) d.partial[n_base_blocks + u] = acc;
-        return;
-    }
-    const int c = bx - n_row_blocks;
-    if (c >= 2 * (S + 1)) return;
-    const int g = c >> 1, r = c & 1, P = arr_pos[g];
-    const double hn = H[n_arr + L - 1];
-    double acc = 0.0;
-    for (int e = wave; e < L; e += 4) {
-        const int xe = d.new_start + (r ? L - 1 - e : e);
-        const double* __restrict__ row = d.M2 + (int64_t)xe * d.ld2;
-#pragma unroll 4
-        for (int q = lane; q < n_arr; q += 64) {
-            const int dd = q < P ? (P + e - q) : (q + L - (P + e));
-            acc += row[p[q]] * (hn - H[dd - 1]);
-        }
-        for (int e2 = e + 1 + lane; e2 < L; e2 += 64) {
-            const int x2 = d.new_start + (r ? L - 1 - e2 : e2);
-            acc += row[x2] * (hn - H[e2 - e - 1]);
-        }
-    }
-    const double sum = block_sum_256(acc, s_w);
-    if (threadIdx.x == 0) d.partial[n_base_blocks + n_arr + c] = sum;
-}
-
-void launch_insb_fast(const InsStep* steps, int n_chrom, int max_S, int max_n_arr, int n_base_blocks, hipStream_t s)
-{
-    const size_t lds = perm_lds_bytes(max_n_arr);
+            for (int q = lane; q < n_arr; q += 64) {
+                const int dd = q < P ? (P + e - q) : (q + L - (P + e));
+                acc += row[p[q]] * (hn - H[dd - 1]);
+            }
+            for (int e2 = e + 1 + lane; e2 < L; e2 += 64) {
+                const int x2 = d.new_start + (r ? L - 1 - e2 : e2);
+                acc += row[x2] * (hn - H[e2 - e - 1]);
+            }
+        }
+        const double sum = block_sum_256(acc, s_w);
+        if (threadIdx.x == 0) put(d.partial + n_base_blocks + n_arr + c, sum);
+    }
+    if (!TAIL) return;
+    const int n_rows_here = (n_arr + 3) / 4;
+    const int expect = n_base_here + n_rows_here + 2 * (S + 1) + count_off;
+    const int k = bx < 0 ? (int)blockIdx.x : (bx < n_row_blocks ? n_base_here + bx : n_base_here + n_rows_here + (bx - n_row_blocks));
+    if (!draw_last_ticket(d.tick, d.tick + 2 * INS_TICK_LINE, k, expect, &s_last)) return;
+    const int now = insb_shortlist_body(d, d.st, reinterpret_cast<double*>(smem), lds_doubles, n_base_blocks, near_top, max_c);
+    if (threadIdx.x == 0) s_last = now;
+    __syncthreads();
+    if (s_last) insb_apply_all(d, d.st);
+}
+
+__global__ __launch_bounds__(256) __attribute__((amdgpu_waves_per_eu(8))) void k_insb_fast(const InsStep* __restrict__ steps, int n_base_blocks, int n_row_blocks,
+                                                   int n_cross_blocks, double near_top, int max_c, int count_off, int lds_doubles)
+{
+    extern __shared__ __attribute__((aligned(16))) unsigned char smem[];
+    insb_fast_pass<true>(steps[blockIdx.y], smem, n_base_blocks, n_row_blocks, n_cross_blocks, near_top, max_c, count_off,
+                         lds_doubles);
+}
+
+__global__ __launch_bounds__(256) void k_insb_fast_unfused(const InsStep* __restrict__ steps, int n_base_blocks, int n_row_blocks,
+                                                           int n_cross_blocks)
+{
+    extern __shared__ __attribute__((aligned(16))) unsigned char smem[];
+    insb_fast_pass<false>(steps[blockIdx.y], smem, n_base_blocks, n_row_blocks, n_cross_blocks, 0.0, 0, 0, 0);
+}
+
+static size_t insb_fast_lds_bytes(int max_S, int max_n_arr, int n_base_blocks, bool tail)
+{
+    const size_t perm = perm_lds_bytes(max_n_arr);
+    if (!tail) return perm;
+    const size_t list = ((((size_t)(max_S + 1) + n_base_blocks) * sizeof(double)) + 15) & ~(size_t)15;
+    const size_t full = list + ((((size_t)(max_n_arr < SL_STAGE_MAX ? max_n_arr : SL_STAGE_MAX) * sizeof(double)) + 15) & ~(size_t)15);
+    const size_t eighth = 160 * 1024 / 8 - 512;
+    size_t lds = list > perm ? list : perm;
+    if (full > lds && full <= eighth) lds = full;
+    return lds;
+}
+
+void launch_insb_fast(const InsStep* steps, int n_chrom, int max_S, int max_n_arr, int n_base_blocks, bool tail, double near_top,
+                      int max_c, int count_off, hipStream_t s)
+{
     const int n_row_blocks = (max_n_arr + 3) / 4, n_cross_blocks = 2 * (max_S + 1);
     static const bool split = getenv("HICMI_P2_INSB_SPLIT") != nullptr;
+    if (split) tail = false;
+    const size_t lds = insb_fast_lds_bytes(max_S, max_n_arr, n_base_blocks, tail);
+    if (getenv("HICMI_PART2_PROFILE")) {
+        static std::atomic<int> told{0};
+        if (!told.exchange(1)) {
+            for (const int n : {2000, 8192}) {
+                int with_tail = 0, without = 0;
+                (void)hipOccupancyMaxActiveBlocksPerMultiprocessor(&with_tail, reinterpret_cast<const void*>(k_insb_fast), 256,
+                                                                   insb_fast_lds_bytes(max_S, n, n_base_blocks, true));
+                (void)hipOccupancyMaxActiveBlocksPerMultiprocessor(&without, reinterpret_cast<const void*>(k_insb_fast_unfused), 256, perm_lds_bytes(n));
+                fprintf(stderr, "[hicmi] k_insb_fast workgroups per CU at max_n_arr %d (max_S %d): %d with its tail, %d without\n", n, max_S, with_tail, without);
+            }
+        }
+    }
     if (split) {
         ensure_dynamic_lds(reinterpret_cast<const void*>(k_insb_base), g_lds_insb_base, lds);
         hipLaunchKernelGGL(k_insb_base, dim3(n_base_blocks, n_chrom), dim3(256), lds, s, steps, n_base_blocks);
     }
-    ensure_dynamic_lds(reinterpret_cast<const void*>(k_insb_fast), g_lds_insb_fast, lds);
-    hipLaunchKernelGGL(k_insb_fast, dim3(n_row_blocks + n_cross_blocks + (split ? 0 : n_base_blocks), n_chrom), dim3(256), lds, s,
-                       steps, n_base_blocks, n_row_blocks, n_cross_blocks);
+    const dim3 grid(n_row_blocks + n_cross_blocks + (split ? 0 : n_base_blocks), n_chrom);
+    if (tail) {
+        ensure_dynamic_lds(reinterpret_cast<const void*>(k_insb_fast), g_lds_insb_fast, lds);
+        hipLaunchKernelGGL(k_insb_fast, grid, dim3(256), lds, s, steps, n_base_blocks, n_row_blocks, n_cross_blocks, near_top,
+                           insb_clamp_max_c(max_c), count_off, (int)(lds / sizeof(double)));
+    } else {
+        ensure_dynamic_lds(reinterpret_cast<const void*>(k_insb_fast_unfused), g_lds_insb_fast_unfused, lds);
+        hipLaunchKernelGGL(k_insb_fast_unfused, grid, dim3(256), lds, s, steps, n_base_blocks, n_row_blocks, n_cross_blocks);
+    }
 }
 
 static constexpr int G_TILE = 2048;
```

Result: slower. 113,100 (-9.0%).
